# ntampellini/TSCoDe

Measured on AMD Instinct MI355X. Metric: conformers/sec, 100k x 50-atom prune_conformers pipeline (embed -> clash mask -> RMSD prune), higher is better.
Workload: dtype f64

## Files before the change

### tscode_amd/csrc/adjacent.hip

```cpp
#include "host.hpp"
#include "call.hpp"
#include "embed_transform.hpp"
#include "scan_kernels.hpp"
#include "gather_rows.hpp"
#include "prune_api.hpp"
#include "group_filter.hpp"
#include "csearch_kernels.hpp"
#include "tfd_kernels.hpp"
#include "moi_kernels.hpp"
#include "host_order.hpp"
#include "trimolecular.hpp"
#include "embed_prune_plan.hpp"

#include <memory>


extern "C" __attribute__((visibility("default"))) int tsc_greedy_group_filter_dev(tsc_ctx *c, const double *poses, const int32_t *group_off_dev, int n_groups,
                                                                             int64_t n_poses, int n_atoms, double rmsd_thr, uint8_t *accepted) {
    TSC_API_GUARD_BEGIN
    TSC_REQUIRE(c && poses && group_off_dev && accepted, "tsc_greedy_group_filter_dev: null argument");
    TSC_REQUIRE(n_groups >= 0 && n_poses >= 0 && n_atoms > 0 && rmsd_thr > 0, "bad sizes");
    if (n_groups == 0 || n_poses == 0) return 0;
    DeviceGuard guard(c->device);
    Scratch s(c);
    double *G;
    TSC_TRY(s.get(size_t(n_poses), &G));
    hipLaunchKernelGGL(k_greedy_group_filter, dim3(n_groups), dim3(256), 0, c->stream, poses, group_off_dev, n_groups, n_atoms, rmsd_thr,
                       accepted, G);
    TSC_HIP(hipGetLastError());
    return 0;
    TSC_API_GUARD_END
}

extern "C" __attribute__((visibility("default"))) int tsc_greedy_group_filter(tsc_ctx *c, const double *poses, const int32_t *group_off, int n_groups, int n_atoms,
                                                                         double rmsd_thr, uint8_t *accepted) {
    TSC_API_GUARD_BEGIN
    TSC_REQUIRE(c && poses && group_off && accepted, "tsc_greedy_group_filter: null argument");
    TSC_REQUIRE(n_groups >= 0 && n_atoms > 0 && rmsd_thr > 0, "bad sizes");
    if (n_groups == 0) return 0;
    TSC_REQUIRE(group_off[0] == 0, "group_off must start at 0");
    for (int g = 0; g < n_groups; ++g)
        TSC_REQUIRE(group_off[g + 1] >= group_off[g] && group_off[g + 1] - group_off[g] <= GF_MAX_GROUP,
                    "group %d: sizes must be in [0, %d]", g, GF_MAX_GROUP);
    const int64_t n_poses = group_off[n_groups];
    if (n_poses == 0) return 0;
    HostCall h(c);
    double *d_poses;
    int32_t *d_off;
    uint8_t *d_acc;
    TSC_TRY(h.in(poses, size_t(n_poses) * n_atoms * 3, &d_poses));
    TSC_TRY(h.in(group_off, size_t(n_groups) + 1, &d_off));
    TSC_TRY(h.out(accepted, size_t(n_poses), &d_acc));
    TSC_TRY(tsc_greedy_group_filter_dev(c, d_poses, d_off, n_groups, n_poses, n_atoms, rmsd_thr, d_acc));
    return h.finish();
    TSC_API_GUARD_END
}


static int csearch_args(int n_atoms, int n_tors, int64_t n_cand, double thresh, int64_t max_clashes, CsearchArgs *a) {
    TSC_REQUIRE(n_atoms > 0 && n_tors >= 0 && n_cand >= 0, "bad sizes (%d atoms, %d torsions, %lld candidates)", n_atoms, n_tors, (long long)n_cand);
    TSC_REQUIRE(n_atoms <= 65535 && torsion_lists_bytes(n_tors, n_atoms) + csearch_wave_bytes(n_atoms) <= 150 * 1024,
                "%d atoms x %d torsions exceed the LDS staging of the csearch kernels", n_atoms, n_tors);
    a->n = n_atoms, a->n_tors = n_tors, a->n_cand = n_cand;
    a->sq_bound = clash_sq_bound(thresh), a->max_clashes = max_clashes;
    return 0;
}

static int csearch_waves(int n_atoms, int n_tors, size_t *lds) {
    int w = 4;
    while (w > 1 && torsion_lists_bytes(n_tors, n_atoms) + w * csearch_wave_bytes(n_atoms) > 150 * 1024) w >>= 1;
    *lds = torsion_lists_bytes(n_tors, n_atoms) + w * csearch_wave_bytes(n_atoms);
    return w;
}

static int check_torsions(const int32_t *torsions, int n_tors, int n_atoms) {
    for (int t = 0; t < n_tors; ++t)
        for (int q = 0; q < 4; ++q)
            TSC_REQUIRE(torsions[4 * t + q] >= 0 && torsions[4 * t + q] < n_atoms, "torsion %d: atom index %d out of range", t, torsions[4 * t + q]);
    return 0;
}

extern "C" __attribute__((visibility("default"))) int tsc_csearch_rotate_dev(tsc_ctx *c, const double *coords, int n_atoms, const int32_t *torsions,
                                                                             const uint8_t *masks, int n_tors, const int32_t *angles, int64_t n_cand,
                                                                             double thresh, int64_t max_clashes, double *out, int32_t *rotated_bonds) {
    TSC_API_GUARD_BEGIN
    TSC_REQUIRE(c && coords && out && rotated_bonds && torsions && masks && angles, "tsc_csearch_rotate_dev: null argument");
    CsearchArgs a;
    TSC_TRY(csearch_args(n_atoms, n_tors, n_cand, thresh, max_clashes, &a));
    if (n_cand == 0) return 0;
    DeviceGuard guard(c->device);
    size_t lds;
    const int waves = csearch_waves(n_atoms, n_tors, &lds);
    TSC_TRY(lds_attribute(&k_csearch_rotate, lds));
    hipLaunchKernelGGL(k_csearch_rotate, dim3(grid_for(n_cand, waves, 256 * 8)), dim3(64 * waves), lds, c->stream, a, coords, torsions, masks, angles, out,
                       rotated_bonds);
    TSC_HIP(hipGetLastError());
    return 0;
    TSC_API_GUARD_END
}

extern "C" __attribute__((visibility("default"))) int tsc_csearch_rotate(tsc_ctx *c, const double *coords, int n_atoms, const int32_t *torsions,
                                                                         const uint8_t *masks, int n_tors, const int32_t *angles, int64_t n_cand,
                                                                         double thresh, int64_t max_clashes, double *out, int32_t *rotated_bonds) {
    TSC_API_GUARD_BEGIN
    TSC_REQUIRE(c && coords && out && rotated_bonds && (n_tors == 0 || (torsions && masks && angles)), "tsc_csearch_rotate: null argument");
    TSC_REQUIRE(n_atoms > 0 && n_tors >= 0 && n_cand >= 0, "bad sizes");
    TSC_TRY(check_torsions(torsions, n_tors, n_atoms));
    if (n_cand == 0) return 0;
    HostCall h(c);
    double *d_coords, *d_out;
    int32_t *d_tors, *d_angles, *d_rb;
    uint8_t *d_masks;
    TSC_TRY(h.in(coords, size_t(n_atoms) * 3, &d_coords));
    TSC_TRY(h.in(torsions, size_t(n_tors) * 4, &d_tors));
    TSC_TRY(h.in(masks, size_t(n_tors) * n_atoms, &d_masks));
    TSC_TRY(h.in(angles, size_t(n_cand) * n_tors, &d_angles));
    TSC_TRY(h.out(out, size_t(n_cand) * n_atoms * 3, &d_out));
    TSC_TRY(h.out(rotated_bonds, size_t(n_cand), &d_rb));
    TSC_TRY(tsc_csearch_rotate_dev(c, d_coords, n_atoms, d_tors, d_masks, n_tors, d_angles, n_cand, thresh, max_clashes, d_out, d_rb));
    return h.finish();
    TSC_API_GUARD_END
}

static int csearch_multi_sets(int n_atoms, const int32_t *set_off, int n_sets, int *t_widest) {
    TSC_REQUIRE(n_atoms > 0 && n_sets > 0 && set_off && set_off[0] == 0, "bad sizes (%d atoms, %d torsion sets; set_off must start at 0)", n_atoms, n_sets);
    int widest = 0;
    for (int k = 0; k < n_sets; ++k) {
        const int t = set_off[k + 1] - set_off[k];
        TSC_REQUIRE(t >= 0, "torsion set %d: set_off must not decrease", k);
        TSC_REQUIRE(n_atoms <= 65535 && torsion_lists_bytes(t, n_atoms) + csearch_wave_bytes(n_atoms) <= 150 * 1024,
                    "torsion set %d: %d atoms x %d torsions exceed the LDS staging of the csearch kernels", k, n_atoms, t);
        widest = std::max(widest, t);
    }
    *t_widest = widest;
    return 0;
}

extern "C" __attribute__((visibility("default"))) int tsc_csearch_multi_plan(const int32_t *cand_start, int64_t n_cand, const int32_t *start_set, int n_starts,
                                                                             const int32_t *set_off, int n_sets, int n_atoms, int32_t *items,
                                                                             int64_t items_cap, int64_t *n_items) {
    TSC_API_GUARD_BEGIN
    TSC_REQUIRE(n_items && (n_cand == 0 || cand_start) && (n_starts == 0 || start_set), "tsc_csearch_multi_plan: null argument");
    TSC_REQUIRE(n_cand >= 0 && n_cand < INT32_MAX && n_starts >= 0, "bad sizes (%lld candidates, %d starts)", (long long)n_cand, n_starts);
    int widest;
    TSC_TRY(csearch_multi_sets(n_atoms, set_off, n_sets, &widest));
    for (int s = 0; s < n_starts; ++s) TSC_REQUIRE(start_set[s] >= 0 && start_set[s] < n_sets, "start %d: torsion set %d out of range", s, start_set[s]);
    size_t lds;
    const int waves = csearch_waves(n_atoms, widest, &lds);
    int64_t count = 0;
    for (int64_t lo = 0; lo < n_cand;) {
        const int s = cand_start[lo];
        TSC_REQUIRE(s >= 0 && s < n_starts && (lo == 0 || s >= cand_start[lo - 1]), "candidate %lld: start %d out of range or out of order", (long long)lo, s);
        const int k = start_set[s];
        int64_t hi = lo + 1;
        while (hi < n_cand && hi - lo < waves && cand_start[hi] >= 0 && cand_start[hi] < n_starts && cand_start[hi] >= cand_start[hi - 1] &&
               start_set[cand_start[hi]] == k)
            ++hi;
        if (items) {
            TSC_REQUIRE(count < items_cap, "tsc_csearch_multi_plan: more than %lld work items", (long long)items_cap);
            items[4 * count] = int32_t(lo), items[4 * count + 1] = int32_t(hi), items[4 * count + 2] = set_off[k], items[4 * count + 3] = set_off[k + 1] - set_off[k];
        }
        ++count, lo = hi;
    }
    *n_items = count;
    return 0;
    TSC_API_GUARD_END
}

extern "C" __attribute__((visibility("default"))) int tsc_csearch_rotate_multi_dev(tsc_ctx *c, const double *starts, int n_atoms, const int32_t *torsions,
                                                                                   const uint8_t *masks, const int32_t *set_off, int n_sets,
                                                                                   const int32_t *angles, int t_max, const int32_t *cand_start,
                                                                                   const int32_t *cand_row, int64_t n_cand, const int32_t *items,
                                                                                   int64_t n_items, double thresh, int64_t max_clashes, double *out,
                                                                                   int32_t *rotated_bonds) {
    TSC_API_GUARD_BEGIN
    TSC_REQUIRE(c && set_off, "tsc_csearch_rotate_multi_dev: null argument");
    int widest;
    TSC_TRY(csearch_multi_sets(n_atoms, set_off, n_sets, &widest));
    TSC_REQUIRE(t_max >= widest && n_items >= 0 && n_items <= n_cand, "bad sizes (table %d wide, widest set %d; %lld work items, %lld candidates)", t_max,
                widest, (long long)n_items, (long long)n_cand);
    CsearchMultiArgs ma;
    TSC_TRY(csearch_args(n_atoms, widest, n_items, thresh, max_clashes, &ma.a));
    TSC_REQUIRE(n_cand < INT32_MAX, "too many candidates");
    if (n_cand == 0) return 0;
    TSC_REQUIRE(starts && out && rotated_bonds && cand_start && cand_row && items && (widest == 0 || (torsions && masks && angles)),
                "tsc_csearch_rotate_multi_dev: null argument");
    DeviceGuard guard(c->device);
    size_t lds;
    const int waves = csearch_waves(n_atoms, widest, &lds);
    ma.t_max = t_max, ma.lists_bytes = torsion_lists_bytes(widest, n_atoms);
    TSC_TRY(lds_attribute(&k_csearch_rotate_multi, lds));
    hipLaunchKernelGGL(k_csearch_rotate_multi, dim3(grid_for(n_items, 1, 256 * 8)), dim3(64 * waves), lds, c->stream, ma, starts, torsions, masks, angles,
                       cand_start, cand_row, items, out, rotated_bonds);
    TSC_HIP(hipGetLastError());
    return 0;
    TSC_API_GUARD_END
}

extern "C" __attribute__((visibility("default"))) int tsc_csearch_rotate_multi(tsc_ctx *c, const double *starts, int n_starts, int n_atoms, const int32_t *torsions,
                                                                               const uint8_t *masks, const int32_t *set_off, int n_sets,
                                                                               const int32_t *start_set, const int32_t *angles, int64_t n_rows, int t_max,
                                                                               const int32_t *cand_start, const int32_t *cand_row, int64_t n_cand,
                                                                               double thresh, int64_t max_clashes, double *out, int32_t *rotated_bonds) {
    TSC_API_GUARD_BEGIN
    TSC_REQUIRE(c && set_off && (n_cand == 0 || (starts && start_set && cand_start && cand_row && out && rotated_bonds)),
                "tsc_csearch_rotate_multi: null argument");
    TSC_REQUIRE(n_starts >= 0 && n_rows >= 0 && n_rows < INT32_MAX && n_cand >= 0 && t_max >= 0, "bad sizes");
    int64_t n_items = 0;
    TSC_TRY(tsc_csearch_multi_plan(cand_start, n_cand, start_set, n_starts, set_off, n_sets, n_atoms, nullptr, 0, &n_items));
    const int n_tors = set_off[n_sets];
    TSC_REQUIRE(n_tors == 0 || (torsions && masks), "tsc_csearch_rotate_multi: null argument");
    TSC_TRY(check_torsions(torsions, n_tors, n_atoms));
    for (int64_t m = 0; m < n_cand; ++m) TSC_REQUIRE(cand_row[m] >= 0 && cand_row[m] < n_rows, "candidate %lld: angle row %d out of range", (long long)m, cand_row[m]);
    if (n_cand == 0) return 0;
    TSC_REQUIRE(n_rows * t_max == 0 || angles, "tsc_csearch_rotate_multi: null argument");
    std::vector<int32_t> items(size_t(n_items) * 4);
    TSC_TRY(tsc_csearch_multi_plan(cand_start, n_cand, start_set, n_starts, set_off, n_sets, n_atoms, items.data(), n_items, &n_items));
    HostCall h(c);
    double *d_starts, *d_out;
    int32_t *d_tors, *d_angles, *d_cs, *d_cr, *d_items, *d_rb;
    uint8_t *d_masks;
    TSC_TRY(h.in(starts, size_t(n_starts) * n_atoms * 3, &d_starts));
    TSC_TRY(h.in(torsions, size_t(n_tors) * 4, &d_tors));
    TSC_TRY(h.in(masks, size_t(n_tors) * n_atoms, &d_masks));
    TSC_TRY(h.in(angles, size_t(n_rows) * t_max, &d_angles));
    TSC_TRY(h.in(cand_start, size_t(n_cand), &d_cs));
    TSC_TRY(h.in(cand_row, size_t(n_cand), &d_cr));
    TSC_TRY(h.in(items.data(), items.size(), &d_items));
    TSC_TRY(h.out(out, size_t(n_cand) * n_atoms * 3, &d_out));
    TSC_TRY(h.out(rotated_bonds, size_t(n_cand), &d_rb));
    TSC_TRY(tsc_csearch_rotate_multi_dev(c, d_starts, n_atoms, d_tors, d_masks, set_off, n_sets, d_angles, t_max, d_cs, d_cr, n_cand, d_items, n_items, thresh,
                                         max_clashes, d_out, d_rb));
    return h.finish();
    TSC_API_GUARD_END
}

extern "C" __attribute__((visibility("default"))) int tsc_csearch_select_dev(tsc_ctx *c, const double *cand, const int32_t *rotated_bonds, int n_atoms,
                                                                             const int32_t *seg_off, const int32_t *seg_start, const int32_t *seg_a0, int n_seg,
                                                                             int n_out, int64_t max_tries, int32_t *kept_count, int32_t *done,
                                                                             int32_t *rows_consumed, double *kept_rows, int64_t capacity,
                                                                             int64_t *n_kept_host) {
    TSC_API_GUARD_BEGIN
    TSC_REQUIRE(c && n_kept_host, "tsc_csearch_select_dev: null argument");
    TSC_REQUIRE(n_atoms > 0 && n_seg >= 0 && capacity >= 0, "bad sizes (%d atoms, %d segments, room for %lld rows)", n_atoms, n_seg, (long long)capacity);
    *n_kept_host = 0;
    if (n_seg == 0) return 0;
    TSC_REQUIRE(cand && rotated_bonds && seg_off && seg_start && seg_a0 && kept_count && done && rows_consumed && (capacity == 0 || kept_rows),
                "tsc_csearch_select_dev: null argument");
    DeviceGuard guard(c->device);
    Scratch s(c);
    int32_t *seg_kept, *total;
    TSC_TRY(s.get(size_t(n_seg), &seg_kept));
    TSC_TRY(s.get(1, &total));
    hipLaunchKernelGGL(k_csearch_select, dim3(grid_for(n_seg, 4, INT32_MAX)), dim3(256), 0, c->stream, rotated_bonds, seg_off, seg_start, seg_a0, n_seg, n_out,
                       (long long)max_tries, kept_count, done, rows_consumed, seg_kept);
    hipLaunchKernelGGL(k_csearch_compact, dim3(grid_for(n_seg, 4, INT32_MAX)), dim3(256), 0, c->stream, cand, rotated_bonds, seg_off, (const int32_t *)seg_kept,
                       n_seg, n_atoms * 3, (long long)capacity, kept_rows, total);
    TSC_HIP(hipGetLastError());
    int32_t kept = 0;
    TSC_TRY(read_i32(c, total, &kept));
    TSC_REQUIRE(kept <= capacity, "tsc_csearch_select_dev: %d rows kept, room for %lld (the rows past it were not written)", kept, (long long)capacity);
    *n_kept_host = kept;
    return 0;
    TSC_API_GUARD_END
}

extern "C" __attribute__((visibility("default"))) int tsc_rotate_dihedral(tsc_ctx *c, const double *coords, int64_t n_structs, int n_atoms, const int32_t *torsion,
                                                                          const uint8_t *mask, const double *angles, double *out) {
    TSC_API_GUARD_BEGIN
    TSC_REQUIRE(c && coords && torsion && mask && angles && out, "tsc_rotate_dihedral: null argument");
    TSC_REQUIRE(n_structs >= 0 && n_atoms > 0, "bad sizes");
    TSC_REQUIRE(out != coords, "tsc_rotate_dihedral: out must not alias coords");
    for (int q = 1; q <= 2; ++q) TSC_REQUIRE(torsion[q] >= 0 && torsion[q] < n_atoms, "torsion index %d out of range", torsion[q]);
    if (n_structs == 0) return 0;
    HostCall h(c);
    double *d_c, *d_o, *d_a;
    uint8_t *d_m;
    TSC_TRY(h.in(coords, size_t(n_structs) * n_atoms * 3, &d_c));
    TSC_TRY(h.in(angles, size_t(n_structs), &d_a));
    TSC_TRY(h.in(mask, size_t(n_atoms), &d_m));
    TSC_TRY(h.out(out, size_t(n_structs) * n_atoms * 3, &d_o));
    hipLaunchKernelGGL(k_rotate_dihedral, dim3(grid_for(n_structs * n_atoms, 256)), dim3(256), 0, c->stream, (const double *)d_c, n_structs, n_atoms, int(torsion[1]),
                       int(torsion[2]), (const uint8_t *)d_m, (const double *)d_a, d_o);
    TSC_HIP(hipGetLastError());
    return h.finish();
    TSC_API_GUARD_END
}

extern "C" __attribute__((visibility("default"))) int tsc_torsion_comp_check(tsc_ctx *c, const double *coords, int64_t n_structs, int n_atoms,
                                                                             const int32_t *torsion, const uint8_t *mask, double thresh,
                                                                             int64_t max_clashes, int32_t *ok) {
    TSC_API_GUARD_BEGIN
    TSC_REQUIRE(c && coords && torsion && mask && ok, "tsc_torsion_comp_check: null argument");
    CsearchArgs a;
    TSC_TRY(csearch_args(n_atoms, 1, n_structs, thresh, max_clashes, &a));
    TSC_TRY(check_torsions(torsion, 1, n_atoms));
    if (n_structs == 0) return 0;
    HostCall h(c);
    double *d_coords;
    int32_t *d_tors, *d_ok;
    uint8_t *d_mask;
    TSC_TRY(h.in(coords, size_t(n_structs) * n_atoms * 3, &d_coords));
    TSC_TRY(h.in(torsion, size_t(4), &d_tors));
    TSC_TRY(h.in(mask, size_t(n_atoms), &d_mask));
    TSC_TRY(h.out(ok, size_t(n_structs), &d_ok));
    size_t lds;
    const int waves = csearch_waves(n_atoms, 1, &lds);
    TSC_TRY(lds_attribute(&k_torsion_comp_check, lds));
    hipLaunchKernelGGL(k_torsion_comp_check, dim3(grid_for(n_structs, waves, 256 * 8)), dim3(64 * waves), lds, c->stream, a, (const double *)d_coords,
                       (const int32_t *)d_tors, (const uint8_t *)d_mask, d_ok);
    TSC_HIP(hipGetLastError());
    return h.finish();
    TSC_API_GUARD_END
}


extern "C" __attribute__((visibility("default"))) int tsc_torsion_fingerprints(tsc_ctx *c, const double *coords, int64_t n_structs, int n_atoms,
                                                                               const int32_t *quads, int n_quads, float *out) {
    TSC_API_GUARD_BEGIN
    TSC_REQUIRE(c && coords && quads && out, "tsc_torsion_fingerprints: null argument");
    TSC_REQUIRE(n_structs >= 0 && n_atoms > 0 && n_quads >= 0, "bad sizes");
    for (int q = 0; q < 4 * n_quads; ++q) TSC_REQUIRE(quads[q] >= 0 && quads[q] < n_atoms, "quadruplet atom index %d out of range", quads[q]);
    if (n_structs == 0 || n_quads == 0) return 0;
    HostCall h(c);
    double *d_coords;
    int32_t *d_quads;
    float *d_out;
    TSC_TRY(h.in(coords, size_t(n_structs) * n_atoms * 3, &d_coords));
    TSC_TRY(h.in(quads, size_t(n_quads) * 4, &d_quads));
    TSC_TRY(h.out(out, size_t(n_structs) * n_quads, &d_out));
    hipLaunchKernelGGL(k_torsion_fingerprints, dim3(grid_for(n_structs * n_quads, 256, 256 * 8)), dim3(256), 0, c->stream, (const double *)d_coords,
                       n_structs, n_atoms, (const int32_t *)d_quads, n_quads, d_out);
    TSC_HIP(hipGetLastError());
    return h.finish();
    TSC_API_GUARD_END
}

extern "C" __attribute__((visibility("default"))) int tsc_tfd_first_similar(tsc_ctx *c, const float *tf, int64_t n_structs, int n_quads, int64_t d,
                                                                            int64_t k, int64_t num_active, double thresh, int32_t *first) {
    TSC_API_GUARD_BEGIN
    TSC_REQUIRE(c && tf && first, "tsc_tfd_first_similar: null argument");
    if (n_structs == 0) return 0;
    TSC_REQUIRE(n_structs >= 0 && n_quads >= 0 && d > 0 && k > 0 && num_active >= 0 && num_active <= n_structs && d * k <= n_structs,
                "bad pass geometry (n = %lld, d = %lld, k = %lld, active = %lld)", (long long)n_structs, (long long)d, (long long)k, (long long)num_active);
    TSC_REQUIRE(n_structs < INT32_MAX, "too many structures");
    if (n_structs == 0) return 0;
    HostCall h(c);
    float *d_tf;
    int32_t *d_first;
    TSC_TRY(h.in(tf, size_t(n_structs) * n_quads, &d_tf));
    TSC_TRY(h.out(first, size_t(n_structs), &d_first));
    hipLaunchKernelGGL(k_tfd_first_similar, dim3(grid_for(n_structs, 4, 256 * 16)), dim3(256), 0, c->stream, (const float *)d_tf, n_structs, n_quads, d, k,
                       num_active, thresh, d_first);
    TSC_HIP(hipGetLastError());
    return h.finish();
    TSC_API_GUARD_END
}

extern "C" __attribute__((visibility("default"))) int tsc_host_graph_step(const int64_t *rel_i, const int64_t *rel_j, const int64_t *chunk_ptr,
                                                                          const int64_t *chunk_off, const int64_t *chunk_len, int64_t n_chunks,
                                                                          int64_t n_total, uint8_t *keep) {
    TSC_API_GUARD_BEGIN
    TSC_REQUIRE(rel_i && rel_j && chunk_ptr && chunk_off && chunk_len && keep && n_chunks >= 0 && n_total >= 0, "tsc_host_graph_step: bad argument");
    int64_t longest = 0;
    for (int64_t c = 0; c < n_chunks; ++c) {
        TSC_REQUIRE(chunk_ptr[c + 1] >= chunk_ptr[c] && chunk_off[c] >= 0 && chunk_len[c] >= 0 && chunk_off[c] + chunk_len[c] <= n_total,
                    "chunk %lld: bad bounds", (long long)c);
        for (int64_t q = chunk_ptr[c]; q < chunk_ptr[c + 1]; ++q)
            TSC_REQUIRE(rel_i[q] >= 0 && rel_i[q] < chunk_len[c] && rel_j[q] >= 0 && rel_j[q] < chunk_len[c] && rel_i[q] != rel_j[q],
                        "match %lld lies outside its chunk", (long long)q);
        longest = std::max(longest, chunk_len[c]);
    }
    std::vector<int32_t> index_of(size_t(longest), -1);
    for (int64_t c = 0; c < n_chunks; ++c)
        tsc_host::graph_step_chunk(rel_i + chunk_ptr[c], rel_j + chunk_ptr[c], chunk_ptr[c + 1] - chunk_ptr[c], chunk_off[c], keep, index_of);
    return 0;
    TSC_API_GUARD_END
}


extern "C" __attribute__((visibility("default"))) int tsc_inertia_moments(tsc_ctx *c, const double *structures, int64_t n_structs, int n_atoms,
                                                                          const double *masses, double *out) {
    TSC_API_GUARD_BEGIN
    TSC_REQUIRE(c && structures && masses && out && n_structs >= 0 && n_atoms > 0, "tsc_inertia_moments: bad argument");
    if (n_structs == 0) return 0;
    HostCall h(c);
    double *d_s, *d_m, *d_o;
    TSC_TRY(h.in(structures, size_t(n_structs) * n_atoms * 3, &d_s));
    TSC_TRY(h.in(masses, size_t(n_atoms), &d_m));
    TSC_TRY(h.out(out, size_t(n_structs) * 3, &d_o));
    hipLaunchKernelGGL(k_inertia_moments, dim3(grid_for(n_structs, 256, 256 * 8)), dim3(256), 0, c->stream, (const double *)d_s, n_structs, n_atoms,
                       (const double *)d_m, d_o);
    TSC_HIP(hipGetLastError());
    return h.finish();
    TSC_API_GUARD_END
}

extern "C" __attribute__((visibility("default"))) int tsc_moi_first_similar(tsc_ctx *c, const double *moments, int64_t n_structs, double max_deviation,
                                                                            int32_t *first) {
    TSC_API_GUARD_BEGIN
    TSC_REQUIRE(c && moments && first && n_structs >= 0 && n_structs < INT32_MAX, "tsc_moi_first_similar: bad argument");
    if (n_structs == 0) return 0;
    HostCall h(c);
    double *d_m;
    int32_t *d_f;
    TSC_TRY(h.in(moments, size_t(n_structs) * 3, &d_m));
    TSC_TRY(h.out(first, size_t(n_structs), &d_f));
    hipLaunchKernelGGL(k_moi_first_similar, dim3(grid_for(n_structs, 4, 256 * 16)), dim3(256), 0, c->stream, (const double *)d_m, n_structs, max_deviation, d_f);
    TSC_HIP(hipGetLastError());
    return h.finish();
    TSC_API_GUARD_END
}

extern "C" __attribute__((visibility("default"))) int tsc_embed_scores(tsc_ctx *c, const double *structures, int64_t n_structs, int n_atoms,
                                                                       const int32_t *indices, const double *distances, int n_c, float *scores,
                                                                       double *fitness_error) {
    TSC_API_GUARD_BEGIN
    TSC_REQUIRE(c && structures && indices && distances && scores && fitness_error && n_structs >= 0 && n_atoms > 0 && n_c >= 0, "tsc_embed_scores: bad argument");
    for (int64_t q = 0; q < n_structs * n_c * 2; ++q) TSC_REQUIRE(indices[q] >= 0 && indices[q] < n_atoms, "constrained index %d out of range", indices[q]);
    if (n_structs == 0) return 0;
    HostCall h(c);
    double *d_s, *d_d, *d_e;
    int32_t *d_i;
    float *d_sc;
    TSC_TRY(h.in(structures, size_t(n_structs) * n_atoms * 3, &d_s));
    TSC_TRY(h.in(indices, size_t(n_structs) * n_c * 2, &d_i));
    TSC_TRY(h.in(distances, size_t(n_structs) * n_c, &d_d));
    TSC_TRY(h.out(scores, size_t(n_structs), &d_sc));
    TSC_TRY(h.out(fitness_error, size_t(n_structs), &d_e));
    hipLaunchKernelGGL(k_embed_scores, dim3(grid_for(n_structs, 256, 256 * 8)), dim3(256), 0, c->stream, (const double *)d_s, n_structs, n_atoms,
                       (const int32_t *)d_i, (const double *)d_d, n_c, d_sc, d_e);
    TSC_HIP(hipGetLastError());
    return h.finish();
    TSC_API_GUARD_END
}


extern "C" __attribute__((visibility("default"))) int tsc_string_embed_params_dev(tsc_ctx *c, const double *p1, const double *p2, const double *ref_vec,
                                                                                  const double *mol_vec, const int32_t *conf_pair, int64_t n_sites,
                                                                                  const double *angles, int n_angles, double *rot, double *pos,
                                                                                  int32_t *conf_idx) {
    TSC_API_GUARD_BEGIN
    TSC_REQUIRE(c && p1 && p2 && ref_vec && mol_vec && conf_pair && angles && rot && pos && conf_idx, "tsc_string_embed_params_dev: null argument");
    TSC_REQUIRE(n_sites >= 0 && n_angles >= 0, "bad sizes");
    if (n_sites == 0 || n_angles == 0) return 0;
    DeviceGuard guard(c->device);
    hipLaunchKernelGGL(k_string_embed_params, dim3(grid_for(n_sites * n_angles, 256, 256 * 8)), dim3(256), 0, c->stream, p1, p2, ref_vec, mol_vec,
                       conf_pair, n_sites, angles, n_angles, rot, pos, conf_idx);
    TSC_HIP(hipGetLastError());
    return 0;
    TSC_API_GUARD_END
}

extern "C" __attribute__((visibility("default"))) int tsc_string_embed_params(tsc_ctx *c, const double *p1, const double *p2, const double *ref_vec,
                                                                              const double *mol_vec, const int32_t *conf_pair, int64_t n_sites,
                                                                              const double *angles, int n_angles, double *rot, double *pos,
                                                                              int32_t *conf_idx) {
    TSC_API_GUARD_BEGIN
    TSC_REQUIRE(c && p1 && p2 && ref_vec && mol_vec && conf_pair && angles && rot && pos && conf_idx, "tsc_string_embed_params: null argument");
    TSC_REQUIRE(n_sites >= 0 && n_angles >= 0, "bad sizes");
    if (n_sites == 0 || n_angles == 0) return 0;
    HostCall h(c);
    double *d_p1, *d_p2, *d_rv, *d_mv, *d_ang, *d_rot, *d_pos;
    int32_t *d_cp, *d_ci;
    const size_t N = size_t(n_sites) * n_angles;
    TSC_TRY(h.in(p1, size_t(n_sites) * 3, &d_p1));
    TSC_TRY(h.in(p2, size_t(n_sites) * 3, &d_p2));
    TSC_TRY(h.in(ref_vec, size_t(n_sites) * 3, &d_rv));
    TSC_TRY(h.in(mol_vec, size_t(n_sites) * 3, &d_mv));
    TSC_TRY(h.in(conf_pair, size_t(n_sites) * 2, &d_cp));
    TSC_TRY(h.in(angles, size_t(n_angles), &d_ang));
    TSC_TRY(h.out(rot, N * 18, &d_rot));
    TSC_TRY(h.out(pos, N * 6, &d_pos));
    TSC_TRY(h.out(conf_idx, N * 2, &d_ci));
    TSC_TRY(tsc_string_embed_params_dev(c, d_p1, d_p2, d_rv, d_mv, d_cp, n_sites, d_ang, n_angles, d_rot, d_pos, d_ci));
    return h.finish();
    TSC_API_GUARD_END
}

extern "C" __attribute__((visibility("default"))) int tsc_cyclical_embed_params(tsc_ctx *c, const double *start, const double *end,
                                                                                const double *direction, const double *pivot, const double *meanpoint,
                                                                                const double *r0, const double *r1, const int32_t *n_reactive,
                                                                                const double *angle, int64_t n, double *rot, double *pos) {
    TSC_API_GUARD_BEGIN
    TSC_REQUIRE(c && start && end && direction && pivot && meanpoint && r0 && r1 && n_reactive && angle && rot && pos, "tsc_cyclical_embed_params: null argument");
    TSC_REQUIRE(n >= 0, "bad size");
    for (int64_t q = 0; q < n; ++q) TSC_REQUIRE(n_reactive[q] == 1 || n_reactive[q] == 2, "row %lld: n_reactive must be 1 or 2", (long long)q);
    if (n == 0) return 0;
    HostCall h(c);
    const double *host[7] = {start, end, direction, pivot, meanpoint, r0, r1};
    double *dev[7], *d_angle, *d_rot, *d_pos;
    int32_t *d_nr;
    for (int i = 0; i < 7; ++i) TSC_TRY(h.in(host[i], size_t(n) * 3, &dev[i]));
    TSC_TRY(h.in(n_reactive, size_t(n), &d_nr));
    TSC_TRY(h.in(angle, size_t(n), &d_angle));
    TSC_TRY(h.out(rot, size_t(n) * 9, &d_rot));
    TSC_TRY(h.out(pos, size_t(n) * 3, &d_pos));
    hipLaunchKernelGGL(k_cyclical_embed_params, dim3(grid_for(n, 256, 256 * 8)), dim3(256), 0, c->stream, (const double *)dev[0], (const double *)dev[1],
                       (const double *)dev[2], (const double *)dev[3], (const double *)dev[4], (const double *)dev[5], (const double *)dev[6],
                       (const int32_t *)d_nr, (const double *)d_angle, n, d_rot, d_pos);
    TSC_HIP(hipGetLastError());
    return h.finish();
    TSC_API_GUARD_END
}


static int launch_tfd_greedy(tsc_ctx *c, Scratch &s, const float *d_tf, int64_t n, int T, double thresh, uint8_t *d_acc, int32_t *d_list, int32_t *d_nk) {
    TSC_REQUIRE(T <= 12288, "fingerprints of %d torsions: the greedy filter takes up to 12288", T);
    uint8_t *d_flags;
    unsigned long long *d_sim;
    float *d_kfp;
    TSC_TRY(s.get(size_t(TG_SUPER) + TG_WORDS * sizeof(unsigned long long), &d_flags));
    TSC_TRY(s.get(size_t(TG_SUPER) * TG_WORDS, &d_sim));
    TSC_TRY(s.get(std::max<size_t>(size_t(n) * T, 1), &d_kfp));
    int32_t *d_nk_before;
    TSC_TRY(s.get(1, &d_nk_before));
    unsigned long long *d_nz = reinterpret_cast<unsigned long long *>(d_flags + TG_SUPER);
    const size_t lds_pairs = 64 * T <= 12288 ? size_t(64) * std::max(T, 1) * sizeof(float) : 0;
    TSC_HIP(hipMemsetAsync(d_nk, 0, sizeof(int32_t), c->stream));
    for (int64_t base = 0; base < n; base += TG_SUPER) {
        const int nc = int(std::min<int64_t>(TG_SUPER, n - base));
        TSC_HIP(hipMemsetAsync(d_flags, 0, size_t(TG_SUPER) + TG_WORDS * sizeof(unsigned long long), c->stream));
        if (base > 0)
            hipLaunchKernelGGL(k_tfd_greedy_prior, dim3(ceil_div(nc, 256), 64), dim3(256), 0, c->stream, d_tf, base, nc, T, thresh, (const float *)d_kfp,
                               (const int32_t *)d_nk, d_flags);
        hipLaunchKernelGGL(k_tfd_greedy_pairs, dim3(TG_WORDS, ceil_div(nc, 256)), dim3(256), lds_pairs, c->stream, d_tf, base, nc, T, thresh, d_sim, d_nz);
        hipLaunchKernelGGL(k_tfd_greedy_replay, dim3(1), dim3(64), 0, c->stream, (const unsigned long long *)d_sim, (const unsigned long long *)d_nz, base, nc,
                           (const uint8_t *)d_flags, d_acc, d_list, d_nk, d_nk_before);
        if (base + TG_SUPER < n && T > 0)
            hipLaunchKernelGGL(k_tfd_greedy_keep, dim3(1), dim3(256), 0, c->stream, d_tf, T, (const int32_t *)d_list, (const int32_t *)d_nk_before,
                               (const int32_t *)d_nk, d_kfp);
    }
    TSC_HIP(hipGetLastError());
    return 0;
}

extern "C" __attribute__((visibility("default"))) int tsc_tfd_greedy_filter(tsc_ctx *c, const float *tf, int64_t n_structs, int n_quads, double thresh,
                                                                            uint8_t *accepted, int64_t *n_kept) {
    TSC_API_GUARD_BEGIN
    TSC_REQUIRE(c && tf && accepted, "tsc_tfd_greedy_filter: null argument");
    TSC_REQUIRE(n_structs >= 0 && n_structs < INT32_MAX && n_quads >= 0, "bad sizes");
    if (n_kept) *n_kept = 0;
    if (n_structs == 0) return 0;
    int32_t nk = 0;
    HostCall h(c);
    float *d_tf;
    uint8_t *d_acc;
    int32_t *d_list, *d_nk;
    TSC_TRY(h.in(tf, std::max<size_t>(size_t(n_structs) * n_quads, 1), &d_tf));
    TSC_TRY(h.out(accepted, size_t(n_structs), &d_acc));
    TSC_TRY(h.scratch().get(size_t(n_structs), &d_list));
    TSC_TRY(h.scratch().get(1, &d_nk));
    TSC_TRY(launch_tfd_greedy(c, h.scratch(), d_tf, n_structs, n_quads, thresh, d_acc, d_list, d_nk));
    TSC_TRY(h.fetch(&nk, d_nk, 1));
    TSC_TRY(h.finish());
    if (n_kept) *n_kept = nk;
    return 0;
    TSC_API_GUARD_END
}

struct EmbedFiltered {
    int32_t n_pass = 0, n_kept = 0;
    double *structs = nullptr;
    int32_t *act = nullptr;
    int32_t *act2 = nullptr;
    const int32_t *ci = nullptr;
    const double *rot = nullptr, *pos = nullptr;
};

template <typename Filter>
static int embed_filter_front(tsc_ctx *c, HostCall &h, const double *d_frags, const FragTable &ft, const int64_t *frag_off, const int32_t *n_atoms,
                              const int32_t *n_conf, const int32_t *d_ci, const double *d_rot, const double *d_pos, int64_t N, double clash_thresh,
                              int64_t max_clashes, uint8_t *clash_ok, uint8_t *kept, EmbedFiltered *f, Filter filter) {
    hipStream_t st = c->stream;
    Scratch &s = h.scratch();
    const int n = ft.n_total;
    uint8_t *d_mask, *d_kept_full, *d_acc;
    int32_t *bsum, *act, *pos_scan, *total, *act2, *total2;
    TSC_TRY(s.get(size_t(N), &d_mask));
    TSC_TRY(h.out(kept, size_t(N), &d_kept_full));
    TSC_TRY(s.get(scan_bsum_count(N), &bsum));
    TSC_TRY(s.get(size_t(N), &act));
    TSC_TRY(s.get(size_t(N) + 1, &pos_scan));
    TSC_TRY(s.get(1, &total));
    TSC_TRY(s.get(size_t(N), &act2));
    TSC_TRY(s.get(1, &total2));
    TSC_TRY(tsc_embed_clash_mask_dev(c, d_frags, frag_off, n_atoms, n_conf, ft.n_mols, d_ci, d_rot, d_pos, N, clash_thresh, max_clashes, d_mask, nullptr));
    TSC_TRY(scan_mask(st, d_mask, N, bsum, pos_scan, act, nullptr, total));
    TSC_TRY(h.fetch(clash_ok, d_mask, size_t(N)));
    TSC_HIP(hipMemsetAsync(d_kept_full, 0, size_t(N), st));
    f->act = act, f->act2 = act2;
    TSC_TRY(read_i32(c, total, &f->n_pass));
    const int32_t n_pass = f->n_pass;
    if (n_pass > 0) {
        double *d_structs;
        TSC_TRY(s.get(size_t(n_pass) * n * 3, &d_structs));
        TSC_TRY(s.get(size_t(n_pass), &d_acc));
        hipLaunchKernelGGL(k_transform, dim3(grid_for(n_pass, TR_POSES, 256 * 64)), dim3(256), transform_lds_bytes(ft.n_mols), st, d_frags, ft, d_ci, d_rot, d_pos,
                           (const int32_t *)act, int64_t(n_pass), d_structs, (const int32_t *)nullptr, 0, (double *)nullptr, (const int32_t *)nullptr);
        TSC_HIP(hipGetLastError());
        f->structs = d_structs;
        TSC_TRY(filter(d_structs, n_pass, pos_scan, total, d_acc));
        hipLaunchKernelGGL(k_scatter_flags, dim3(grid_for(n_pass, 256, 1024)), dim3(256), 0, st, (const uint8_t *)d_acc, (const int32_t *)act, (const int32_t *)total,
                           d_kept_full);
        TSC_TRY(scan_mask(st, d_acc, n_pass, bsum, nullptr, act2, nullptr, total2));
        TSC_TRY(read_i32(c, total2, &f->n_kept));
    }
    return 0;
}

static int embed_filter_fetch(tsc_ctx *c, HostCall &h, int n, const EmbedFiltered &f, double *poses, int64_t poses_capacity, int64_t *n_kept_out) {
    if (poses && f.n_kept > 0) {
        double *d_out;
        TSC_REQUIRE(f.n_kept <= poses_capacity, "poses holds %lld rows, %d poses were kept", (long long)poses_capacity, f.n_kept);
        TSC_TRY(h.scratch().get(size_t(f.n_kept) * n * 3, &d_out));
        TSC_TRY(launch_gather_rows(c->stream, f.structs, f.act2, f.n_kept, n * 3, nullptr, n * 3, d_out));
        TSC_TRY(h.fetch(poses, d_out, size_t(f.n_kept) * n * 3));
    }
    TSC_TRY(h.finish());
    *n_kept_out = f.n_kept;
    return 0;
}

template <typename Filter>
static int embed_filter_run(tsc_ctx *c, HostCall &h, const double *d_frags, const FragTable &ft, const int64_t *frag_off, const int32_t *n_atoms,
                            const int32_t *n_conf, const int32_t *d_ci, const double *d_rot, const double *d_pos, int64_t N, double clash_thresh,
                            int64_t max_clashes, uint8_t *clash_ok, uint8_t *kept, double *poses, int64_t poses_capacity, int64_t *n_pass_out,
                            int64_t *n_kept_out, Filter filter) {
    EmbedFiltered f;
    const int rc = embed_filter_front(c, h, d_frags, ft, frag_off, n_atoms, n_conf, d_ci, d_rot, d_pos, N, clash_thresh, max_clashes, clash_ok, kept, &f, filter);
    *n_pass_out = f.n_pass;
    TSC_TRY(rc);
    return embed_filter_fetch(c, h, ft.n_total, f, poses, poses_capacity, n_kept_out);
}

extern "C" __attribute__((visibility("default"))) int tsc_string_embed(tsc_ctx *c, const double *frags, const int64_t *frag_off, const int32_t *n_atoms,
                                                                       const int32_t *n_conf, const double *p1, const double *p2, const double *ref_vec,
                                                                       const double *mol_vec, const int32_t *conf_pair, int64_t n_sites, const double *angles,
                                                                       int n_angles, double clash_thresh, int64_t max_clashes, const int32_t *quads, int n_quads,
                                                                       double tfd_thresh, uint8_t *clash_ok, uint8_t *kept, double *poses,
                                                                       int64_t poses_capacity, int64_t *n_pass, int64_t *n_kept) {
    TSC_API_GUARD_BEGIN
    TSC_REQUIRE(c && frags && frag_off && n_atoms && n_conf && p1 && p2 && ref_vec && mol_vec && conf_pair && angles && clash_ok && kept && n_pass && n_kept,
                "tsc_string_embed: null argument");
    TSC_REQUIRE(n_sites >= 0 && n_angles >= 0 && n_quads >= 0 && (n_quads == 0 || quads), "bad sizes");
    const int64_t N = n_sites * n_angles;
    TSC_REQUIRE(N < INT32_MAX, "too many candidates");
    *n_pass = *n_kept = 0;
    if (N == 0) return 0;
    FragTable ft;
    TSC_TRY(make_frag_table(frag_off, n_atoms, n_conf, 2, &ft));
    for (int64_t q = 0; q < n_sites; ++q)
        TSC_REQUIRE(conf_pair[2 * q] >= 0 && conf_pair[2 * q] < n_conf[0] && conf_pair[2 * q + 1] >= 0 && conf_pair[2 * q + 1] < n_conf[1],
                    "site %lld: conformer index out of range", (long long)q);
    for (int q = 0; q < 4 * n_quads; ++q) TSC_REQUIRE(quads[q] >= 0 && quads[q] < ft.n_total, "quadruplet atom index %d out of range", quads[q]);
    HostCall h(c);
    Scratch &s = h.scratch();
    double *d_frags, *d_p1, *d_p2, *d_rv, *d_mv, *d_ang, *d_rot, *d_pos;
    int32_t *d_cp, *d_ci, *d_quads = nullptr;
    TSC_TRY(h.in(frags, size_t(frags_total_doubles(frag_off, n_atoms, n_conf, 2)), &d_frags));
    TSC_TRY(h.in(p1, size_t(n_sites) * 3, &d_p1));
    TSC_TRY(h.in(p2, size_t(n_sites) * 3, &d_p2));
    TSC_TRY(h.in(ref_vec, size_t(n_sites) * 3, &d_rv));
    TSC_TRY(h.in(mol_vec, size_t(n_sites) * 3, &d_mv));
    TSC_TRY(h.in(conf_pair, size_t(n_sites) * 2, &d_cp));
    TSC_TRY(h.in(angles, size_t(n_angles), &d_ang));
    if (n_quads) TSC_TRY(h.in(quads, size_t(n_quads) * 4, &d_quads));
    TSC_TRY(s.get(size_t(N) * 18, &d_rot));
    TSC_TRY(s.get(size_t(N) * 6, &d_pos));
    TSC_TRY(s.get(size_t(N) * 2, &d_ci));
    TSC_TRY(tsc_string_embed_params_dev(c, d_p1, d_p2, d_rv, d_mv, d_cp, n_sites, d_ang, n_angles, d_rot, d_pos, d_ci));
    const int n = ft.n_total;
    auto filter = [&](const double *d_structs, int32_t np, const int32_t *, const int32_t *, uint8_t *d_acc) -> int {
        float *d_tf;
        int32_t *d_list, *d_nk;
        TSC_TRY(s.get(std::max<size_t>(size_t(np) * n_quads, 1), &d_tf));
        TSC_TRY(s.get(size_t(np), &d_list));
        TSC_TRY(s.get(1, &d_nk));
        if (n_quads)
            hipLaunchKernelGGL(k_torsion_fingerprints, dim3(grid_for(int64_t(np) * n_quads, 256, 256 * 8)), dim3(256), 0, c->stream, d_structs, int64_t(np), n,
                               (const int32_t *)d_quads, n_quads, d_tf);
        TSC_HIP(hipGetLastError());
        return launch_tfd_greedy(c, s, d_tf, int64_t(np), n_quads, tfd_thresh, d_acc, d_list, d_nk);
    };
    return embed_filter_run(c, h, d_frags, ft, frag_off, n_atoms, n_conf, d_ci, d_rot, d_pos, N, clash_thresh, max_clashes, clash_ok, kept, poses, poses_capacity,
                            n_pass, n_kept, filter);
    TSC_API_GUARD_END
}

extern "C" __attribute__((visibility("default"))) int tsc_cyclical_embed(tsc_ctx *c, const double *frags, const int64_t *frag_off, const int32_t *n_atoms,
                                                                         const int32_t *n_conf, int n_mols, const double *start, const double *end,
                                                                         const double *direction, const double *pivot, const double *meanpoint, const double *r0,
                                                                         const double *r1, const int32_t *n_reactive, const double *angle, const int32_t *conf_idx,
                                                                         int64_t n_poses, const int32_t *group_off, int n_groups, double clash_thresh,
                                                                         int64_t max_clashes, double rmsd_thr, uint8_t *clash_ok, uint8_t *kept, double *poses,
                                                                         int64_t poses_capacity, int64_t *n_pass, int64_t *n_kept) {
    TSC_API_GUARD_BEGIN
    TSC_REQUIRE(c && frags && frag_off && n_atoms && n_conf && start && end && direction && pivot && meanpoint && r0 && r1 && n_reactive && angle && conf_idx &&
                    group_off && clash_ok && kept && n_pass && n_kept,
                "tsc_cyclical_embed: null argument");
    TSC_REQUIRE(n_poses >= 0 && n_poses < INT32_MAX && n_groups >= 0 && rmsd_thr > 0, "bad sizes");
    *n_pass = *n_kept = 0;
    if (n_poses == 0) return 0;
    FragTable ft;
    TSC_TRY(make_frag_table(frag_off, n_atoms, n_conf, n_mols, &ft));
    const int64_t rows = n_poses * n_mols;
    for (int64_t q = 0; q < rows; ++q) {
        TSC_REQUIRE(n_reactive[q] == 1 || n_reactive[q] == 2, "row %lld: n_reactive must be 1 or 2", (long long)q);
        TSC_REQUIRE(conf_idx[q] >= 0 && conf_idx[q] < n_conf[q % n_mols], "row %lld: conformer index out of range", (long long)q);
    }
    TSC_REQUIRE(n_groups > 0 && group_off[0] == 0 && group_off[n_groups] == n_poses, "group_off must run from 0 to n_poses");
    for (int g = 0; g < n_groups; ++g)
        TSC_REQUIRE(group_off[g + 1] >= group_off[g] && group_off[g + 1] - group_off[g] <= GF_MAX_GROUP, "group %d: sizes must be in [0, %d]", g, GF_MAX_GROUP);
    HostCall h(c);
    Scratch &s = h.scratch();
    const double *host[7] = {start, end, direction, pivot, meanpoint, r0, r1};
    double *d_frags, *dev[7], *d_angle, *d_rot, *d_pos;
    int32_t *d_nr, *d_ci, *d_goff, *d_goff_pass;
    TSC_TRY(h.in(frags, size_t(frags_total_doubles(frag_off, n_atoms, n_conf, n_mols)), &d_frags));
    for (int i = 0; i < 7; ++i) TSC_TRY(h.in(host[i], size_t(rows) * 3, &dev[i]));
    TSC_TRY(h.in(n_reactive, size_t(rows), &d_nr));
    TSC_TRY(h.in(angle, size_t(rows), &d_angle));
    TSC_TRY(h.in(conf_idx, size_t(rows), &d_ci));
    TSC_TRY(h.in(group_off, size_t(n_groups) + 1, &d_goff));
    TSC_TRY(s.get(size_t(n_groups) + 1, &d_goff_pass));
    TSC_TRY(s.get(size_t(rows) * 9, &d_rot));
    TSC_TRY(s.get(size_t(rows) * 3, &d_pos));
    hipLaunchKernelGGL(k_cyclical_embed_params, dim3(grid_for(rows, 256, 256 * 8)), dim3(256), 0, c->stream, (const double *)dev[0], (const double *)dev[1],
                       (const double *)dev[2], (const double *)dev[3], (const double *)dev[4], (const double *)dev[5], (const double *)dev[6],
                       (const int32_t *)d_nr, (const double *)d_angle, rows, d_rot, d_pos);
    TSC_HIP(hipGetLastError());
    const int n = ft.n_total;
    auto filter = [&](const double *d_structs, int32_t np, const int32_t *pos_scan, const int32_t *total, uint8_t *d_acc) -> int {
        hipLaunchKernelGGL(k_group_offsets_after_filter, dim3(grid_for(n_groups + 1, 256, 1024)), dim3(256), 0, c->stream, (const int32_t *)d_goff, n_groups, pos_scan,
                           n_poses, total, d_goff_pass);
        TSC_HIP(hipGetLastError());
        return tsc_greedy_group_filter_dev(c, d_structs, d_goff_pass, n_groups, np, n, rmsd_thr, d_acc);
    };
    return embed_filter_run(c, h, d_frags, ft, frag_off, n_atoms, n_conf, d_ci, d_rot, d_pos, n_poses, clash_thresh, max_clashes, clash_ok, kept, poses,
                            poses_capacity, n_pass, n_kept, filter);
    TSC_API_GUARD_END
}

static int check_group_slab_sizes(int64_t n_groups, int n_angles, double rmsd_thr) {
    TSC_REQUIRE(n_angles >= 1 && n_angles <= GF_MAX_GROUP, "%d angle sets per group: must be in [1, %d]", n_angles, GF_MAX_GROUP);
    TSC_REQUIRE(n_groups >= 0 && n_groups < INT32_MAX / n_angles, "%lld groups of %d poses: too many candidates", (long long)n_groups, n_angles);
    TSC_REQUIRE(rmsd_thr > 0, "bad sizes");
    return 0;
}
static int check_group_slab_records(const int32_t *n_conf, int n_mols, const int32_t *n_reactive, const int32_t *conf_idx, int64_t n_groups) {
    for (int64_t q = 0; q < n_groups * n_mols; ++q) {
        TSC_REQUIRE(n_reactive[q] == 1 || n_reactive[q] == 2, "group %lld, molecule %d: n_reactive must be 1 or 2", (long long)(q / n_mols), int(q % n_mols));
        TSC_REQUIRE(conf_idx[q] >= 0 && conf_idx[q] < n_conf[q % n_mols], "group %lld, molecule %d: conformer index out of range", (long long)(q / n_mols),
                    int(q % n_mols));
    }
    return 0;
}

static int cyclical_groups_front(tsc_ctx *c, HostCall &h, std::vector<int32_t> &goff, const double *d_frags, const FragTable &ft, const int64_t *frag_off,
                                 const int32_t *n_atoms, const int32_t *n_conf, const double *const host[7], const int32_t *n_reactive, const int32_t *conf_idx,
                                 const double *angles, int64_t n_groups, int n_angles, double clash_thresh, int64_t max_clashes, double rmsd_thr,
                                 uint8_t *clash_ok, uint8_t *kept, EmbedFiltered *f) {
    const int n_mols = ft.n_mols;
    const int64_t items = n_groups * n_mols, n_poses = n_groups * n_angles, rows = n_poses * n_mols;
    goff.resize(size_t(n_groups) + 1);
    for (int64_t g = 0; g <= n_groups; ++g) goff[size_t(g)] = int32_t(g * n_angles);
    Scratch &s = h.scratch();
    double *dev[7], *d_angles, *d_rot, *d_pos;
    int32_t *d_nr, *d_cg, *d_ci, *d_goff, *d_goff_pass;
    for (int i = 0; i < 7; ++i) TSC_TRY(h.in(host[i], size_t(items) * 3, &dev[i]));
    TSC_TRY(h.in(n_reactive, size_t(items), &d_nr));
    TSC_TRY(h.in(conf_idx, size_t(items), &d_cg));
    TSC_TRY(h.in(angles, size_t(n_angles) * n_mols, &d_angles));
    TSC_TRY(h.in(goff.data(), size_t(n_groups) + 1, &d_goff));
    TSC_TRY(s.get(size_t(n_groups) + 1, &d_goff_pass));
    TSC_TRY(s.get(size_t(rows) * 9, &d_rot));
    TSC_TRY(s.get(size_t(rows) * 3, &d_pos));
    TSC_TRY(s.get(size_t(rows), &d_ci));
    hipLaunchKernelGGL(k_cyclical_embed_group_params, dim3(grid_for(ceil_div(n_groups, int64_t(64 / n_mols)), CGP_WAVES, 768)), dim3(64 * CGP_WAVES), 0, c->stream,
                       (const double *)dev[0], (const double *)dev[1], (const double *)dev[2], (const double *)dev[3], (const double *)dev[4],
                       (const double *)dev[5], (const double *)dev[6], (const int32_t *)d_nr, (const int32_t *)d_cg, (const double *)d_angles, n_groups, n_mols,
                       n_angles, d_rot, d_pos, d_ci);
    TSC_HIP(hipGetLastError());
    f->ci = d_ci, f->rot = d_rot, f->pos = d_pos;
    const int n = ft.n_total;
    const int ng = int(n_groups);
    auto filter = [&](const double *d_structs, int32_t np, const int32_t *pos_scan, const int32_t *total, uint8_t *d_acc) -> int {
        hipLaunchKernelGGL(k_group_offsets_after_filter, dim3(grid_for(ng + 1, 256, 1024)), dim3(256), 0, c->stream, (const int32_t *)d_goff, ng, pos_scan, n_poses,
                           total, d_goff_pass);
        TSC_HIP(hipGetLastError());
        return tsc_greedy_group_filter_dev(c, d_structs, d_goff_pass, ng, np, n, rmsd_thr, d_acc);
    };
    return embed_filter_front(c, h, d_frags, ft, frag_off, n_atoms, n_conf, d_ci, d_rot, d_pos, n_poses, clash_thresh, max_clashes, clash_ok, kept, f, filter);
}

extern "C" __attribute__((visibility("default"))) int tsc_cyclical_embed_groups(tsc_ctx *c, const double *frags, const int64_t *frag_off, const int32_t *n_atoms,
                                                                                const int32_t *n_conf, int n_mols, const double *start, const double *end,
                                                                                const double *direction, const double *pivot, const double *meanpoint,
                                                                                const double *r0, const double *r1, const int32_t *n_reactive,
                                                                                const int32_t *conf_idx, const double *angles, int64_t n_groups, int n_angles,
                                                                                double clash_thresh, int64_t max_clashes, double rmsd_thr, uint8_t *clash_ok,
                                                                                uint8_t *kept, double *poses, int64_t poses_capacity, int64_t *n_pass,
                                                                                int64_t *n_kept) {
    TSC_API_GUARD_BEGIN
    TSC_REQUIRE(c && frags && frag_off && n_atoms && n_conf && start && end && direction && pivot && meanpoint && r0 && r1 && n_reactive && conf_idx && angles &&
                    clash_ok && kept && n_pass && n_kept,
                "tsc_cyclical_embed_groups: null argument");
    TSC_REQUIRE(n_mols == 2 || n_mols == 3, "tsc_cyclical_embed_groups: %d molecules, the cyclical embed takes 2 or 3", n_mols);
    TSC_TRY(check_group_slab_sizes(n_groups, n_angles, rmsd_thr));
    *n_pass = *n_kept = 0;
    if (n_groups == 0) return 0;
    FragTable ft;
    TSC_TRY(make_frag_table(frag_off, n_atoms, n_conf, n_mols, &ft));
    TSC_TRY(check_group_slab_records(n_conf, n_mols, n_reactive, conf_idx, n_groups));
    std::vector<int32_t> goff;
    HostCall h(c);
    const double *host[7] = {start, end, direction, pivot, meanpoint, r0, r1};
    double *d_frags;
    TSC_TRY(h.in(frags, size_t(frags_total_doubles(frag_off, n_atoms, n_conf, n_mols)), &d_frags));
    EmbedFiltered f;
    const int rc = cyclical_groups_front(c, h, goff, d_frags, ft, frag_off, n_atoms, n_conf, host, n_reactive, conf_idx, angles, n_groups, n_angles, clash_thresh,
                                         max_clashes, rmsd_thr, clash_ok, kept, &f);
    *n_pass = f.n_pass;
    TSC_TRY(rc);
    return embed_filter_fetch(c, h, ft.n_total, f, poses, poses_capacity, n_kept);
    TSC_API_GUARD_END
}


static thread_local float g_trimolecular_ms = -1.f;

extern "C" __attribute__((visibility("default"))) int tsc_trimolecular_groups_timings(tsc_ctx *c, float *ms) {
    TSC_API_GUARD_BEGIN
    TSC_REQUIRE(c && ms, "tsc_trimolecular_groups_timings: null argument");
    *ms = g_trimolecular_ms;
    return 0;
    TSC_API_GUARD_END
}

extern "C" __attribute__((visibility("default"))) int tsc_trimolecular_groups(
    tsc_ctx *c, const double *frags, const int64_t *frag_off, const int32_t *n_atoms, const int32_t *n_conf, const int32_t *reactive, const int32_t *n_reactive,
    const int64_t *reactive_cumnums, const int32_t *n_rows, const int32_t *conf, const double *pivot, const double *meanpoint, const int64_t *cumnums,
    const double *tri_poly, const double *tri_cost, const double *directions, const uint8_t *mask, const int64_t *base, int64_t n_triples, int64_t n_groups,
    double *blocks, int64_t *group_ids, int32_t *best) {
    TSC_API_GUARD_BEGIN
    TSC_REQUIRE(c && frags && frag_off && n_atoms && n_conf && reactive && n_reactive && reactive_cumnums && n_rows, "tsc_trimolecular_groups: null argument");
    TSC_REQUIRE(n_triples >= 0 && n_groups >= 0 && n_groups < INT32_MAX, "tsc_trimolecular_groups: %lld triples, %lld groups", (long long)n_triples,
                (long long)n_groups);
    FragTable ft;
    TSC_TRY(make_frag_table(frag_off, n_atoms, n_conf, 3, &ft));
    TriTables tb;
    memset(&tb, 0, sizeof(tb));
    const int64_t *row = reactive_cumnums;
    for (int m = 0; m < 3; ++m) {
        tb.frag_off[m] = frag_off[m], tb.n_atoms[m] = n_atoms[m], tb.n_reactive[m] = n_reactive[m], tb.n_rows[m] = n_rows[m];
        TSC_REQUIRE(n_reactive[m] == 1 || n_reactive[m] == 2, "tsc_trimolecular_groups: molecule %d has %d reactive atoms, must be 1 or 2", m, n_reactive[m]);
        for (int k = 0; k < n_reactive[m]; ++k) {
            TSC_REQUIRE(reactive[2 * m + k] >= 0 && reactive[2 * m + k] < n_atoms[m], "tsc_trimolecular_groups: reactive atom %d of molecule %d with %d atoms",
                        reactive[2 * m + k], m, n_atoms[m]);
            tb.reactive[m][k] = reactive[2 * m + k];
        }
        TSC_REQUIRE(n_rows[m] >= 0 && n_rows[m] <= TG_MAX_ROWS, "tsc_trimolecular_groups: molecule %d has %d reactive_cumnums rows, at most %d are taken", m,
                    n_rows[m], TG_MAX_ROWS);
        for (int r = 0; r < n_rows[m]; ++r, row += 2) {
            TSC_REQUIRE(row[0] >= 0 && row[0] < n_atoms[m], "tsc_trimolecular_groups: reactive_cumnums row %d of molecule %d names atom %lld of %d", r, m,
                        (long long)row[0], n_atoms[m]);
            tb.row_atom[m][r] = int(row[0]), tb.row_cum[m][r] = row[1];
        }
    }
    g_trimolecular_ms = -1.f;
    if (n_triples == 0) {
        TSC_REQUIRE(n_groups == 0, "tsc_trimolecular_groups: %lld groups from no triple", (long long)n_groups);
        return 0;
    }
    TSC_REQUIRE(conf && pivot && meanpoint && cumnums && tri_poly && tri_cost && directions && mask && base, "tsc_trimolecular_groups: null argument");
    TSC_REQUIRE(n_groups == 0 || (blocks && group_ids && best), "tsc_trimolecular_groups: null output");
    int64_t running = 0;
    for (int64_t t = 0; t < n_triples; ++t) {
        TSC_REQUIRE(base[t] == running, "tsc_trimolecular_groups: triple %lld: base %lld, the orientation masks in front of it count %lld", (long long)t,
                    (long long)base[t], (long long)running);
        running += __builtin_popcount(mask[t]);
        for (int m = 0; m < 3; ++m)
            TSC_REQUIRE(conf[3 * t + m] >= 0 && conf[3 * t + m] < n_conf[m], "tsc_trimolecular_groups: triple %lld, molecule %d: conformer %d of %d",
                        (long long)t, m, conf[3 * t + m], n_conf[m]);
        if (!mask[t]) continue;
        for (int q = 0; q < 6; ++q) {
            bool found = false;
            for (int m = 0; m < 3 && !found; ++m)
                for (int r = 0; r < tb.n_rows[m] && !found; ++r) found = tb.row_cum[m][r] == cumnums[6 * t + q];
            TSC_REQUIRE(found, "tsc_trimolecular_groups: triple %lld: cumnum %lld of molecule %d's pivot is in no molecule's reactive_cumnums", (long long)t,
                        (long long)cumnums[6 * t + q], q / 2);
        }
    }
    TSC_REQUIRE(running == n_groups, "tsc_trimolecular_groups: the orientation masks count %lld groups, n_groups is %lld", (long long)running, (long long)n_groups);
    if (n_groups == 0) return 0;
    HostCall h(c);
    const size_t T = size_t(n_triples), G = size_t(n_groups);
    const double *d_frags, *d_pivot, *d_mean, *d_poly, *d_cost, *d_dir;
    const int32_t *d_conf;
    const int64_t *d_cum, *d_base;
    const uint8_t *d_mask;
    double *d_blocks;
    int64_t *d_ids;
    int32_t *d_best;
    TSC_TRY(h.in(frags, size_t(frags_total_doubles(frag_off, n_atoms, n_conf, 3)), &d_frags));
    TSC_TRY(h.in(conf, T * 3, &d_conf));
    TSC_TRY(h.in(pivot, T * 9, &d_pivot));
    TSC_TRY(h.in(meanpoint, T * 9, &d_mean));
    TSC_TRY(h.in(cumnums, T * 6, &d_cum));
    TSC_TRY(h.in(tri_poly, T * 9, &d_poly));
    TSC_TRY(h.in(tri_cost, T * 9, &d_cost));
    TSC_TRY(h.in(directions, T * 9, &d_dir));
    TSC_TRY(h.in(mask, T, &d_mask));
    TSC_TRY(h.in(base, T, &d_base));
    TSC_TRY(h.out(blocks, G * 3 * TG_RECORD, &d_blocks));
    TSC_TRY(h.out(group_ids, G * 6, &d_ids));
    TSC_TRY(h.out(best, G, &d_best));
    StageTimer tm(c);
    tm.begin();
    hipLaunchKernelGGL(k_trimolecular_groups, dim3(grid_for(n_triples, TG_WAVES, 512)), dim3(64 * TG_WAVES), 0, c->stream, d_frags, tb, d_conf, d_pivot, d_mean,
                       d_cum, d_poly, d_cost, d_dir, d_mask, d_base, n_triples, d_blocks, d_ids, d_best);
    const hipError_t launched = hipGetLastError();
    if (launched == hipSuccess) tm.end(&g_trimolecular_ms);
    TSC_HIP(launched);
    return h.finish();
    TSC_API_GUARD_END
}


struct tsc_embed_prune : Owned {
    using Owned::Owned;
    FragTable ft{};
    int64_t frag_off[MAX_MOLS] = {};
    int32_t n_atoms[MAX_MOLS] = {}, n_conf[MAX_MOLS] = {};
    int n_heavy = 0;
    double *frags = nullptr;
    int32_t *sel = nullptr;
    double *heavy = nullptr, *rot = nullptr, *pos = nullptr;
    int32_t *ci = nullptr;
    uint8_t *survived = nullptr;
    int64_t cap = 0, n_kept = 0, n_survived = 0;
    bool pruned = false;
};

static __global__ __launch_bounds__(256) void k_kept_candidates(const int32_t *__restrict__ act, const int32_t *__restrict__ act2, int n_kept,
                                                                int32_t *__restrict__ cand) {
    for (int r = blockIdx.x * 256 + threadIdx.x; r < n_kept; r += gridDim.x * 256) cand[r] = act[act2[r]];
}

static __global__ __launch_bounds__(256) void k_gather_rows_i32(const int32_t *__restrict__ src, const int32_t *__restrict__ idx, int64_t n_out, int row,
                                                                int32_t *__restrict__ dst) {
    const int64_t total = n_out * row;
    for (int64_t e = int64_t(blockIdx.x) * 256 + threadIdx.x; e < total; e += int64_t(gridDim.x) * 256) {
        const int64_t r = e / row;
        dst[e] = src[int64_t(idx[r]) * row + (e - r * row)];
    }
}

static int embed_prune_reserve(tsc_embed_prune *r, int64_t need) {
    tsc_ctx *c = r->ctx;
    const int64_t cap = ep_grown_capacity(r->cap, need);
    TSC_REQUIRE(cap >= 0, "tsc_embed_prune_add_groups: %lld kept poses are more than a prune takes (%lld)", (long long)need, (long long)EP_MAX_ROWS);
    if (cap == r->cap) return 0;
    const int nm = r->ft.n_mols;
    const size_t row_bytes[4] = {size_t(r->n_heavy) * 24, size_t(nm) * 72, size_t(nm) * 24, size_t(nm) * 4};
    void *old[4] = {r->heavy, r->rot, r->pos, r->ci}, *grown[4] = {nullptr, nullptr, nullptr, nullptr};
    int rc = 0;
    for (int i = 0; i < 4 && !rc; ++i) rc = r->take(size_t(cap) * row_bytes[i], &grown[i]);
    for (int i = 0; i < 4 && !rc; ++i)
        if (r->n_kept > 0 && hipMemcpyAsync(grown[i], old[i], size_t(r->n_kept) * row_bytes[i], hipMemcpyDeviceToDevice, c->stream) != hipSuccess)
            rc = fail(TSC_ERR_HIP, "tsc_embed_prune_add_groups: the copy into the grown buffers failed");
    void *const *gone = rc ? grown : old;
    for (int i = 0; i < 4; ++i) r->give_back(gone[i]);
    if (rc) return rc;
    r->heavy = static_cast<double *>(grown[0]), r->rot = static_cast<double *>(grown[1]), r->pos = static_cast<double *>(grown[2]);
    r->ci = static_cast<int32_t *>(grown[3]);
    r->cap = cap;
    return 0;
}

extern "C" __attribute__((visibility("default"))) int tsc_embed_prune_destroy(tsc_embed_prune *r) {
    TSC_API_GUARD_BEGIN
    return destroy_owned(r);
    TSC_API_GUARD_END
}

extern "C" __attribute__((visibility("default"))) int tsc_embed_prune_create(tsc_ctx *c, const double *frags, const int64_t *frag_off, const int32_t *n_atoms,
                                                                             const int32_t *n_conf, int n_mols, const int32_t *heavy_idx, int n_heavy,
                                                                             tsc_embed_prune **out) {
    TSC_API_GUARD_BEGIN
    TSC_REQUIRE(c && frags && frag_off && n_atoms && n_conf && heavy_idx && out, "tsc_embed_prune_create: null argument");
    *out = nullptr;
    TSC_REQUIRE(n_mols == 2 || n_mols == 3, "tsc_embed_prune_create: %d molecules, the cyclical embed takes 2 or 3", n_mols);
    FragTable ft;
    TSC_TRY(make_frag_table(frag_off, n_atoms, n_conf, n_mols, &ft));
    TSC_REQUIRE(n_heavy >= 1 && n_heavy <= ft.n_total, "tsc_embed_prune_create: %d heavy atoms of %d atoms: at least one, at most all", n_heavy, ft.n_total);
    std::vector<int32_t> sel(size_t(n_heavy) * 3);
    for (int a = 0; a < n_heavy; ++a) {
        TSC_REQUIRE(heavy_idx[a] >= 0 && heavy_idx[a] < ft.n_total, "tsc_embed_prune_create: heavy_idx[%d] = %d is not an atom of the %d", a, heavy_idx[a],
                    ft.n_total);
        TSC_REQUIRE(a == 0 || heavy_idx[a] > heavy_idx[a - 1], "tsc_embed_prune_create: heavy_idx[%d] = %d does not increase", a, heavy_idx[a]);
        for (int k = 0; k < 3; ++k) sel[size_t(a) * 3 + k] = heavy_idx[a] * 3 + k;
    }
    HostCall h(c);
    std::unique_ptr<tsc_embed_prune> run(new tsc_embed_prune(c));
    run->ft = ft, run->n_heavy = n_heavy;
    for (int m = 0; m < n_mols; ++m) run->frag_off[m] = frag_off[m], run->n_atoms[m] = n_atoms[m], run->n_conf[m] = n_conf[m];
    TSC_TRY(h.in(frags, size_t(frags_total_doubles(frag_off, n_atoms, n_conf, n_mols)), &run->frags));
    TSC_TRY(h.in(sel.data(), sel.size(), &run->sel));
    TSC_TRY(h.finish());
    run->take_blocks(h.scratch());
    c->owned.adopt(run.get());
    *out = run.release();
    return 0;
    TSC_API_GUARD_END
}

extern "C" __attribute__((visibility("default"))) int tsc_embed_prune_add_groups(tsc_embed_prune *r, const double *start, const double *end, const double *direction,
                                                                                 const double *pivot, const double *meanpoint, const double *r0, const double *r1,
                                                                                 const int32_t *n_reactive, const int32_t *conf_idx, const double *angles,
                                                                                 int64_t n_groups, int n_angles, double clash_thresh, int64_t max_clashes,
                                                                                 double rmsd_thr_filter, uint8_t *clash_ok, uint8_t *kept, int64_t *n_pass,
                                                                                 int64_t *n_kept) {
    TSC_API_GUARD_BEGIN
    TSC_REQUIRE(r && start && end && direction && pivot && meanpoint && r0 && r1 && n_reactive && conf_idx && angles && clash_ok && kept && n_pass && n_kept,
                "tsc_embed_prune_add_groups: null argument");
    if (r->pruned) return fail(TSC_ERR_STATE, "tsc_embed_prune_add_groups: the run has been pruned (tsc_embed_prune_run); a further slab needs a new run");
    TSC_TRY(check_group_slab_sizes(n_groups, n_angles, rmsd_thr_filter));
    *n_pass = *n_kept = 0;
    if (n_groups == 0) return 0;
    tsc_ctx *c = r->ctx;
    const int n_mols = r->ft.n_mols, n = r->ft.n_total;
    TSC_TRY(check_group_slab_records(r->n_conf, n_mols, n_reactive, conf_idx, n_groups));
    std::vector<int32_t> goff;
    HostCall h(c);
    const double *host[7] = {start, end, direction, pivot, meanpoint, r0, r1};
    EmbedFiltered f;
    const int rc = cyclical_groups_front(c, h, goff, r->frags, r->ft, r->frag_off, r->n_atoms, r->n_conf, host, n_reactive, conf_idx, angles, n_groups, n_angles,
                                         clash_thresh, max_clashes, rmsd_thr_filter, clash_ok, kept, &f);
    *n_pass = f.n_pass;
    TSC_TRY(rc);
    if (f.n_kept > 0) {
        TSC_TRY(embed_prune_reserve(r, r->n_kept + f.n_kept));
        int32_t *cand;
        TSC_TRY(h.scratch().get(size_t(f.n_kept), &cand));
        hipLaunchKernelGGL(k_kept_candidates, dim3(grid_for(f.n_kept, 256, 1024)), dim3(256), 0, c->stream, (const int32_t *)f.act, (const int32_t *)f.act2, f.n_kept,
                           cand);
        TSC_HIP(hipGetLastError());
        const int64_t at = r->n_kept;
        TSC_TRY(launch_gather_rows(c->stream, f.structs, f.act2, f.n_kept, n * 3, r->sel, r->n_heavy * 3, r->heavy + ep_row_offset(at, r->n_heavy * 3)));
        TSC_TRY(launch_gather_rows(c->stream, f.rot, cand, f.n_kept, n_mols * 9, nullptr, n_mols * 9, r->rot + ep_row_offset(at, n_mols * 9)));
        TSC_TRY(launch_gather_rows(c->stream, f.pos, cand, f.n_kept, n_mols * 3, nullptr, n_mols * 3, r->pos + ep_row_offset(at, n_mols * 3)));
        hipLaunchKernelGGL(k_gather_rows_i32, dim3(grid_for(int64_t(f.n_kept) * n_mols, 256, 1024)), dim3(256), 0, c->stream, f.ci, (const int32_t *)cand,
                           int64_t(f.n_kept), n_mols, r->ci + ep_row_offset(at, n_mols));
        TSC_HIP(hipGetLastError());
    }
    TSC_TRY(h.finish());
    r->n_kept += f.n_kept;
    *n_kept = f.n_kept;
    return 0;
    TSC_API_GUARD_END
}

extern "C" __attribute__((visibility("default"))) int tsc_embed_prune_count(tsc_embed_prune *r, int64_t *n_kept_total) {
    TSC_API_GUARD_BEGIN
    TSC_REQUIRE(r && n_kept_total, "tsc_embed_prune_count: null argument");
    *n_kept_total = r->n_kept;
    return 0;
    TSC_API_GUARD_END
}

extern "C" __attribute__((visibility("default"))) int tsc_embed_prune_run(tsc_embed_prune *r, double rmsd_thr, int mode, uint8_t *survived, tsc_pass_stats *stats,
                                                                          int *n_passes, int64_t *n_survived) {
    TSC_API_GUARD_BEGIN
    TSC_REQUIRE(r && n_survived && (survived || r->n_kept == 0), "tsc_embed_prune_run: null argument");
    TSC_REQUIRE(mode == 0 || mode == 1, "tsc_embed_prune_run: mode %d (0: reference-exact, 1: cache-free)", mode);
    TSC_REQUIRE(rmsd_thr > 0, "tsc_embed_prune_run: rmsd_thr = %g must be positive", rmsd_thr);
    *n_survived = 0;
    if (n_passes) *n_passes = 0;
    tsc_ctx *c = r->ctx;
    if (r->n_kept == 0) {
        r->pruned = true, r->n_survived = 0;
        return 0;
    }
    DeviceGuard guard(c->device);
    if (!r->survived) TSC_TRY(r->get(size_t(r->n_kept), &r->survived));
    r->pruned = true, r->n_survived = 0;
    TSC_TRY(tsc_prune_rmsd_dev(c, r->heavy, r->n_kept, r->n_heavy, rmsd_thr, mode, r->survived, stats, n_passes));
    TSC_HIP(hipMemcpyAsync(survived, r->survived, size_t(r->n_kept), hipMemcpyDeviceToHost, c->stream));
    TSC_HIP(hipStreamSynchronize(c->stream));
    int64_t count = 0;
    for (int64_t i = 0; i < r->n_kept; ++i) count += survived[i] != 0;
    r->n_survived = count;
    *n_survived = count;
    return 0;
    TSC_API_GUARD_END
}

extern "C" __attribute__((visibility("default"))) int tsc_embed_prune_poses(tsc_embed_prune *r, int which, double *poses, int64_t capacity) {
    TSC_API_GUARD_BEGIN
    TSC_REQUIRE(r && poses, "tsc_embed_prune_poses: null argument");
    TSC_REQUIRE(which == 0 || which == 1, "tsc_embed_prune_poses: which = %d (0: the survivors, 1: every kept pose)", which);
    if (which == 0 && !r->pruned) return fail(TSC_ERR_STATE, "tsc_embed_prune_poses: the survivors are known once tsc_embed_prune_run has run");
    const int64_t rows = which == 0 ? r->n_survived : r->n_kept;
    TSC_REQUIRE(capacity >= rows, "tsc_embed_prune_poses: poses holds %lld rows, %lld are asked for", (long long)capacity, (long long)rows);
    if (rows == 0) return 0;
    tsc_ctx *c = r->ctx;
    const int n = r->ft.n_total;
    HostCall h(c);
    Scratch &s = h.scratch();
    int32_t *act = nullptr;
    if (which == 0) {
        int32_t *bsum;
        TSC_TRY(s.get(scan_bsum_count(r->n_kept), &bsum));
        TSC_TRY(s.get(size_t(r->n_kept), &act));
        TSC_TRY(scan_mask(c->stream, r->survived, r->n_kept, bsum, nullptr, act, nullptr, nullptr));
    }
    double *d_out;
    TSC_TRY(s.get(size_t(rows) * n * 3, &d_out));
    hipLaunchKernelGGL(k_transform, dim3(grid_for(rows, TR_POSES, 256 * 64)), dim3(256), transform_lds_bytes(r->ft.n_mols), c->stream, (const double *)r->frags, r->ft,
                       (const int32_t *)r->ci, (const double *)r->rot, (const double *)r->pos, (const int32_t *)act, rows, d_out, (const int32_t *)nullptr, 0,
                       (double *)nullptr, (const int32_t *)nullptr);
    TSC_HIP(hipGetLastError());
    TSC_TRY(h.fetch(poses, (const double *)d_out, size_t(rows) * n * 3));
    return h.finish();
    TSC_API_GUARD_END
}
```

### tscode_amd/csrc/describe.hpp

```cpp
#pragma once
#include "descriptor.hpp"
#include "embed_clash.hpp"

namespace tsc {

__device__ inline void describe_from_lds(const double *s_q, const double *s_x, int pitch, int h, int nf0, int nf1, const double *__restrict__ bias,
                                         int ns, int S, int64_t i0, float *__restrict__ D, double *__restrict__ G, unsigned *__restrict__ dmax_bits) {
    const int T = 256 / S;
    const int sidx = threadIdx.x / T, sub = threadIdx.x - sidx * T;
    const bool mine = sidx < ns;
    double d[DW], g = 0.0;
#pragma unroll
    for (int k = 0; k < DW; ++k) d[k] = 0.0;
    if (mine) {
        const double *x = s_x + sidx * pitch;
        const double *q1 = s_q + KD * nf0;
        for (int a = sub; a < h; a += T) {
            const double n2 = x[3 * a] * x[3 * a] + x[3 * a + 1] * x[3 * a + 1] + x[3 * a + 2] * x[3 * a + 2];
            g += n2;
            if (a < nf0) {
                const double f = sqrt(n2);
#pragma unroll
                for (int k = 0; k < KD; ++k) d[k] = fma(s_q[k * nf0 + a], f, d[k]);
            }
            if (a < nf1) {
                const double f = feature(x, h, 1, a);
#pragma unroll
                for (int k = 0; k < KD; ++k) d[KD + k] = fma(q1[k * nf1 + a], f, d[KD + k]);
            }
        }
    }
    for (int off = T >> 1; off > 0; off >>= 1) {
#pragma unroll
        for (int k = 0; k < DW; ++k) d[k] += __shfl_xor(d[k], off);
        g += __shfl_xor(g, off);
    }
    float mx = 0.0f;
    if (mine && sub == 0) {
        float v[DW];
#pragma unroll
        for (int k = 0; k < DW; ++k) {
            v[(k % KD) * 2 + k / KD] = float(d[k] - bias[k]);
            mx = fmaxf(mx, fabsf(float(d[k] - bias[k])));
        }
        f32x4 *dst = reinterpret_cast<f32x4 *>(D + (i0 + sidx) * DW);
#pragma unroll
        for (int k = 0; k < DW / 4; ++k) dst[k] = f32x4{v[4 * k], v[4 * k + 1], v[4 * k + 2], v[4 * k + 3]};
        G[i0 + sidx] = g;
    }
    for (int off = 32; off > 0; off >>= 1) mx = fmaxf(mx, __shfl_xor(mx, off));
    if ((threadIdx.x & 63) == 0 && mx > __uint_as_float(__hip_atomic_load(dmax_bits, __ATOMIC_RELAXED, __HIP_MEMORY_SCOPE_AGENT)))
        atomicMax(dmax_bits, __float_as_uint(mx));
    if (__ballot(mine && sub == 0 && !(g < 1.7976931348623157e308)) != 0 && (threadIdx.x & 63) == 0) atomicMax(dmax_bits, NONFINITE_BITS);
}

inline __global__ __launch_bounds__(256) void k_descriptors(const double *__restrict__ heavy, int64_t n, int h, int nf0, int nf1,
                                                      const double *__restrict__ Q, const double *__restrict__ bias, float *__restrict__ D,
                                                      double *__restrict__ G, unsigned *__restrict__ dmax_bits, int S) {
    extern __shared__ __attribute__((aligned(16))) double s_mem[];
    const int h3 = h * 3, pitch = h3 | 1;
    double *s_q = s_mem, *s_x = s_mem + KD * (nf0 + nf1);
    for (int e = threadIdx.x; e < KD * (nf0 + nf1); e += 256) s_q[e] = Q[e];
    const int64_t i0 = int64_t(blockIdx.x) * S;
    const int ns = int(min<int64_t>(S, n - i0));
    const double *src = heavy + i0 * h3;
    for (int base = threadIdx.x; base < ns * h3; base += 256 * 8) {
        double v[8];
#pragma unroll
        for (int j = 0; j < 8; ++j) v[j] = (base + 256 * j < ns * h3) ? src[base + 256 * j] : 0.0;
#pragma unroll
        for (int j = 0; j < 8; ++j) {
            const int e = base + 256 * j;
            if (e < ns * h3) {
                const int row = e / h3;
                s_x[row * pitch + (e - row * h3)] = v[j];
            }
        }
    }
    __syncthreads();
    describe_from_lds(s_q, s_x, pitch, h, nf0, nf1, bias, ns, S, i0, D, G, dmax_bits);
}

inline __global__ __launch_bounds__(256) void k_transform_describe(const double *__restrict__ frags, FragTable ft, const int32_t *__restrict__ conf_idx,
                                                             const double *__restrict__ rot, const double *__restrict__ pos,
                                                             const int32_t *__restrict__ idx, double *__restrict__ out,
                                                             const int32_t *__restrict__ heavy_slot, int n_heavy, double *__restrict__ heavy_out,
                                                             const int32_t *__restrict__ n_out_dev, int nf0, int nf1, const double *__restrict__ Q,
                                                             const double *__restrict__ bias, float *__restrict__ D, double *__restrict__ G,
                                                             unsigned *__restrict__ dmax_bits, float *__restrict__ heavy32_out = nullptr) {
    extern __shared__ __attribute__((aligned(16))) double s_tr[];
    const int n = ft.n_total, nm = ft.n_mols, tid = threadIdx.x, pitch = (n_heavy * 3) | 1;
    const int pitch32 = heavy32_pitch(n_heavy), pad32 = pitch32 - 3 * n_heavy;
    const int64_t n_out = *n_out_dev;
    int64_t *sP = reinterpret_cast<int64_t *>(s_tr);
    double *sR = s_tr + TR_POSES, *sT = sR + TR_POSES * nm * 9;
    int *sC = reinterpret_cast<int *>(sT + TR_POSES * nm * 3);
    double *s_q = s_tr + (transform_lds_bytes(nm) + 15) / 16 * 2, *s_x = s_q + KD * (nf0 + nf1);
    for (int e = tid; e < KD * (nf0 + nf1); e += 256) s_q[e] = Q[e];
    for (int64_t r0 = int64_t(blockIdx.x) * TR_POSES; r0 < n_out; r0 += int64_t(gridDim.x) * TR_POSES) {
        const int np = int(min<int64_t>(TR_POSES, n_out - r0));
        if (tid < np) sP[tid] = int64_t(idx[r0 + tid]);
        __syncthreads();
        for (int q = tid; q < np * nm * 9; q += 256) {
            const int row = q / (nm * 9), w = q - row * nm * 9;
            sR[q] = rot[sP[row] * nm * 9 + w];
        }
        for (int q = tid; q < np * nm * 3; q += 256) {
            const int row = q / (nm * 3), w = q - row * nm * 3;
            sT[q] = pos[sP[row] * nm * 3 + w];
        }
        for (int q = tid; q < np * nm; q += 256) {
            const int row = q / nm, w = q - row * nm;
            sC[q] = conf_idx[sP[row] * nm + w];
        }
        __syncthreads();
        for (int e = tid; e < np * n; e += 256) {
            const int row = e / n, a = e - row * n;
            const int64_t r = r0 + row;
            double v[3];
            embed_atom_staged(frags, ft, sR, sT, sC, row, a, v);
            if (out) {
                double *o = out + (r * n + a) * 3;
                o[0] = v[0], o[1] = v[1], o[2] = v[2];
            }
            const int hs = heavy_slot[a];
            if (hs >= 0) {
                double *hv = heavy_out + (r * n_heavy + hs) * 3, *x = s_x + row * pitch + hs * 3;
                hv[0] = x[0] = v[0], hv[1] = x[1] = v[1], hv[2] = x[2] = v[2];
                if (heavy32_out) {
                    float *hf = heavy32_out + r * pitch32 + hs * 3;
                    hf[0] = float(v[0]), hf[1] = float(v[1]), hf[2] = float(v[2]);
                }
            }
        }
        if (heavy32_out)
            for (int e = tid; e < np * pad32; e += 256) heavy32_out[(r0 + e / pad32) * pitch32 + 3 * n_heavy + e % pad32] = 0.0f;
        __syncthreads();
        describe_from_lds(s_q, s_x, pitch, n_heavy, nf0, nf1, bias, np, TR_POSES, r0, D, G, dmax_bits);
        __syncthreads();
    }
}

inline size_t transform_describe_lds_bytes(int n_mols, int h) {
    return (transform_lds_bytes(n_mols) + 15) / 16 * 16 + (size_t(KD) * (n_features(h, 0) + n_features(h, 1)) + size_t(TR_POSES) * ((h * 3) | 1)) * sizeof(double);
}

}
```

### tscode_amd/csrc/embed.hip

```cpp
#include "host.hpp"
#include "call.hpp"
#include "embed_transform.hpp"
#include "embed_clash_kernels.hpp"
#include "scan_kernels.hpp"
#include "gather_rows.hpp"


extern "C" __attribute__((visibility("default"))) int tsc_transform_batch_dev(tsc_ctx *c, const double *frags, const int64_t *frag_off, const int32_t *n_atoms,
                                       const int32_t *n_conf, int n_mols, const int32_t *conf_idx, const double *rot,
                                       const double *pos, int64_t n_poses, double *out) {
    TSC_API_GUARD_BEGIN
    TSC_REQUIRE(c && frags && conf_idx && rot && pos && out, "tsc_transform_batch_dev: null argument");
    TSC_REQUIRE(n_poses >= 0, "negative n_poses");
    FragTable ft;
    TSC_TRY(make_frag_table(frag_off, n_atoms, n_conf, n_mols, &ft));
    if (n_poses == 0) return 0;
    DeviceGuard guard(c->device);
    hipLaunchKernelGGL(k_transform, dim3(grid_for(n_poses, TR_POSES, 256 * 64)), dim3(256), transform_lds_bytes(ft.n_mols), c->stream, frags, ft, conf_idx, rot,
                       pos, (const int32_t *)nullptr, n_poses, out, (const int32_t *)nullptr, 0, (double *)nullptr, (const int32_t *)nullptr);
    TSC_HIP(hipGetLastError());
    return 0;
    TSC_API_GUARD_END
}


extern "C" __attribute__((visibility("default"))) int tsc_transform_batch(tsc_ctx *c, const double *frags, const int64_t *frag_off, const int32_t *n_atoms,
                                   const int32_t *n_conf, int n_mols, const int32_t *conf_idx, const double *rot,
                                   const double *pos, int64_t n_poses, double *out) {
    TSC_API_GUARD_BEGIN
    TSC_REQUIRE(c && frags && conf_idx && rot && pos && out, "tsc_transform_batch: null argument");
    FragTable ft;
    TSC_TRY(make_frag_table(frag_off, n_atoms, n_conf, n_mols, &ft));
    TSC_REQUIRE(n_poses >= 0, "negative n_poses");
    for (int64_t i = 0; i < n_poses * n_mols; ++i)
        TSC_REQUIRE(conf_idx[i] >= 0 && conf_idx[i] < n_conf[i % n_mols], "conf_idx[%lld] out of range", (long long)i);
    if (n_poses == 0) return 0;
    HostCall h(c);
    double *d_frags, *d_rot, *d_pos, *d_out;
    int32_t *d_ci;
    TSC_TRY(h.in(frags, size_t(frags_total_doubles(frag_off, n_atoms, n_conf, n_mols)), &d_frags));
    TSC_TRY(h.in(conf_idx, size_t(n_poses) * n_mols, &d_ci));
    TSC_TRY(h.in(rot, size_t(n_poses) * n_mols * 9, &d_rot));
    TSC_TRY(h.in(pos, size_t(n_poses) * n_mols * 3, &d_pos));
    TSC_TRY(h.out(out, size_t(n_poses) * ft.n_total * 3, &d_out));
    TSC_TRY(tsc_transform_batch_dev(c, d_frags, frag_off, n_atoms, n_conf, n_mols, d_ci, d_rot, d_pos, n_poses, d_out));
    return h.finish();
    TSC_API_GUARD_END
}


static int make_clash_args(int64_t n_poses, int n_atoms, const int32_t *ids, int n_ids, double thresh, int64_t max_clashes,
                           ClashArgs *a) {
    TSC_REQUIRE(n_poses >= 0 && n_atoms > 0, "bad sizes");
    TSC_REQUIRE(n_ids == 0 || n_ids == 2 || n_ids == 3, "ids must have 0 (None), 2 or 3 entries, got %d", n_ids);
    memset(a, 0, sizeof(*a));
    a->n_poses = n_poses;
    a->n = n_atoms;
    a->max_clashes = max_clashes;
    if (n_ids == 0) {
        a->self_mode = 1;
        a->first_row = 0;
        a->n_mols = 1;
        a->sq_bound = clash_sq_bound(0.5);
        for (int m = 1; m <= MAX_MOLS; ++m) a->atom_off[m] = n_atoms;
    } else {
        TSC_REQUIRE(ids != nullptr, "ids is null");
        int off = 0;
        for (int m = 0; m < n_ids; ++m) {
            a->atom_off[m] = off;
            TSC_REQUIRE(ids[m] >= 0, "negative fragment length");
            off += ids[m];
        }
        TSC_REQUIRE(off - ids[n_ids - 1] <= n_atoms, "fragment lengths exceed the atom count");
        for (int m = n_ids; m <= MAX_MOLS; ++m) a->atom_off[m] = n_atoms;
        a->n_mols = n_ids;
        a->first_row = a->atom_off[1];
        a->sq_bound = clash_sq_bound(thresh);
    }
    int rows = std::max(1, n_atoms - a->first_row);
    a->lp = std::min(64, std::max(4, pow2_ceil(rows)));
    return 0;
}

template <bool FUSED, bool SELF, bool MINMODE>
static int launch_clash_impl(tsc_ctx *c, const ClashArgs &a, const double *coords, const double *frags, const FragTable &ft,
                             const int32_t *conf_idx, const double *rot, const double *pos, uint8_t *mask, int32_t *counts) {
    const int ppw = 64 / a.lp;
    size_t lds = size_t(4) * clash_lds_per_wave(a.n, a.lp, MINMODE);
    TSC_REQUIRE(lds <= 160 * 1024, "pose too large for the LDS staging of the clash kernel (%d atoms)", a.n);
    int64_t waves = ceil_div<int64_t>(a.n_poses, ppw);
    int blocks = grid_for(waves, 4, 256 * 32);
    TSC_TRY(lds_attribute(&k_clash<FUSED, SELF, MINMODE>, lds));
    hipLaunchKernelGGL((k_clash<FUSED, SELF, MINMODE>), dim3(blocks), dim3(256), lds, c->stream, a, coords, frags, ft, conf_idx, rot, pos, mask, counts);
    TSC_HIP(hipGetLastError());
    return 0;
}

template <bool FUSED>
static int launch_clash(tsc_ctx *c, const ClashArgs &a, const double *coords, const double *frags, const FragTable &ft,
                        const int32_t *conf_idx, const double *rot, const double *pos, uint8_t *mask, int32_t *counts) {
    if (a.n_poses == 0) return 0;
    if (a.self_mode) return launch_clash_impl<FUSED, true, false>(c, a, coords, frags, ft, conf_idx, rot, pos, mask, counts);
    const bool minmode = !counts && a.max_clashes == 0 && c->opt.clash_fp32 != 0 && 4 * clash_lds_per_wave(a.n, a.lp, true) <= 160 * 1024;
    if (minmode && FUSED && c->opt.clash_lanes != 0 && a.n_mols == 2 && ft.n_mols == 2 && a.atom_off[1] == ft.atom_off[1] && a.n == ft.n_total &&
        std::min(ft.n_atoms[0], ft.n_atoms[1]) >= 1 && std::min(ft.n_atoms[0], ft.n_atoms[1]) <= 32) {
        const int mA = ft.n_atoms[0] <= ft.n_atoms[1] ? 0 : 1, mB = 1 - mA, na2 = (ft.n_atoms[mA] + 1) / 2;
        const dim3 grid(unsigned(grid_for(ceil_div<int64_t>(a.n_poses, 64), 4, 256 * 32)));
#define TSC_LAUNCH_CLASH_LANES(N)                                                                                                          \
    hipLaunchKernelGGL(k_clash_lanes<N>, grid, dim3(256), 0, c->stream, a.n_poses, frags, ft, mA, mB, conf_idx, rot, pos, a.sq_bound, mask)
        if (na2 <= 4) TSC_LAUNCH_CLASH_LANES(4);
        else if (na2 <= 8) TSC_LAUNCH_CLASH_LANES(8);
        else if (na2 <= 12) TSC_LAUNCH_CLASH_LANES(12);
        else if (na2 <= 13) TSC_LAUNCH_CLASH_LANES(13);
        else TSC_LAUNCH_CLASH_LANES(16);
#undef TSC_LAUNCH_CLASH_LANES
        TSC_HIP(hipGetLastError());
        return 0;
    }
    if (minmode && FUSED && c->opt.clash_lanes != 0 && (a.n_mols == 2 || a.n_mols == 3) && ft.n_mols == a.n_mols && a.n == ft.n_total &&
        a.atom_off[1] == ft.atom_off[1] && (a.n_mols == 2 || a.atom_off[2] == ft.atom_off[2])) {
        auto cost = [&](int na2) {
            int64_t w = 0;
            const int n_pairs = a.n_mols == 2 ? 1 : 3;
            for (int pr = 0; pr < n_pairs; ++pr) {
                const int mA = a.n_mols == 2 ? 1 : (pr == 0 ? 1 : (pr == 1 ? 2 : 0)), mB = a.n_mols == 2 ? 0 : (pr == 0 ? 0 : (pr == 1 ? 1 : 2));
                const int64_t tiles = ceil_div(ft.n_atoms[mA], 2 * na2);
                w += tiles * ft.n_atoms[mB] * (2 * na2 + 4);
            }
            return w;
        };
        int best = 12;
        for (int na2 : {16, 18})
            if (cost(na2) < cost(best)) best = na2;
        const dim3 grid(unsigned(grid_for(ceil_div<int64_t>(a.n_poses, CLM_POSES), 1, 256 * 32)));
#define TSC_LAUNCH_CLASH_MULTI(N)                                                                                                          \
    hipLaunchKernelGGL(k_clash_lanes_multi<N>, grid, dim3(256), 0, c->stream, a.n_poses, frags, ft, conf_idx, rot, pos, a.sq_bound, mask)
        if (best == 12) TSC_LAUNCH_CLASH_MULTI(12);
        else if (best == 16) TSC_LAUNCH_CLASH_MULTI(16);
        else TSC_LAUNCH_CLASH_MULTI(18);
#undef TSC_LAUNCH_CLASH_MULTI
        TSC_HIP(hipGetLastError());
        return 0;
    }
    if (minmode) return launch_clash_impl<FUSED, false, true>(c, a, coords, frags, ft, conf_idx, rot, pos, mask, counts);
    return launch_clash_impl<FUSED, false, false>(c, a, coords, frags, ft, conf_idx, rot, pos, mask, counts);
}

extern "C" __attribute__((visibility("default"))) int tsc_clash_mask_dev(tsc_ctx *c, const double *coords, int64_t n_poses, int n_atoms, const int32_t *ids, int n_ids,
                                  double thresh, int64_t max_clashes, uint8_t *mask, int32_t *counts) {
    TSC_API_GUARD_BEGIN
    TSC_REQUIRE(c && coords && mask, "tsc_clash_mask_dev: null argument");
    ClashArgs a;
    TSC_TRY(make_clash_args(n_poses, n_atoms, ids, n_ids, thresh, max_clashes, &a));
    DeviceGuard guard(c->device);
    FragTable ft;
    memset(&ft, 0, sizeof(ft));
    return launch_clash<false>(c, a, coords, nullptr, ft, nullptr, nullptr, nullptr, mask, counts);
    TSC_API_GUARD_END
}

extern "C" __attribute__((visibility("default"))) int tsc_clash_mask(tsc_ctx *c, const double *coords, int64_t n_poses, int n_atoms, const int32_t *ids, int n_ids,
                              double thresh, int64_t max_clashes, uint8_t *mask, int32_t *counts) {
    TSC_API_GUARD_BEGIN
    TSC_REQUIRE(c && coords && mask, "tsc_clash_mask: null argument");
    ClashArgs a;
    TSC_TRY(make_clash_args(n_poses, n_atoms, ids, n_ids, thresh, max_clashes, &a));
    if (n_poses == 0) return 0;
    HostCall h(c);
    double *d_coords;
    uint8_t *d_mask;
    int32_t *d_counts;
    TSC_TRY(h.in(coords, size_t(n_poses) * n_atoms * 3, &d_coords));
    TSC_TRY(h.out(mask, size_t(n_poses), &d_mask));
    TSC_TRY(h.out(counts, size_t(n_poses), &d_counts));
    TSC_TRY(tsc_clash_mask_dev(c, d_coords, n_poses, n_atoms, ids, n_ids, thresh, max_clashes, d_mask, d_counts));
    return h.finish();
    TSC_API_GUARD_END
}

extern "C" __attribute__((visibility("default"))) int tsc_embed_clash_mask_dev(tsc_ctx *c, const double *frags, const int64_t *frag_off, const int32_t *n_atoms,
                                        const int32_t *n_conf, int n_mols, const int32_t *conf_idx, const double *rot,
                                        const double *pos, int64_t n_poses, double thresh, int64_t max_clashes, uint8_t *mask,
                                        int32_t *counts) {
    TSC_API_GUARD_BEGIN
    TSC_REQUIRE(c && frags && conf_idx && rot && pos && mask, "tsc_embed_clash_mask_dev: null argument");
    TSC_REQUIRE(n_mols == 2 || n_mols == 3, "the fused embed+clash path needs 2 or 3 fragments, got %d", n_mols);
    FragTable ft;
    TSC_TRY(make_frag_table(frag_off, n_atoms, n_conf, n_mols, &ft));
    ClashArgs a;
    TSC_TRY(make_clash_args(n_poses, ft.n_total, n_atoms, n_mols, thresh, max_clashes, &a));
    DeviceGuard guard(c->device);
    return launch_clash<true>(c, a, nullptr, frags, ft, conf_idx, rot, pos, mask, counts);
    TSC_API_GUARD_END
}

extern "C" __attribute__((visibility("default"))) int tsc_all_dists(tsc_ctx *c, const double *A, int na, const double *B, int nb, double *out) {
    TSC_API_GUARD_BEGIN
    TSC_REQUIRE(c && A && B && out && na >= 0 && nb >= 0, "tsc_all_dists: bad argument");
    if (na == 0 || nb == 0) return 0;
    HostCall h(c);
    double *dA, *dB, *dO;
    TSC_TRY(h.in(A, size_t(na) * 3, &dA));
    TSC_TRY(h.in(B, size_t(nb) * 3, &dB));
    TSC_TRY(h.out(out, size_t(na) * nb, &dO));
    hipLaunchKernelGGL(k_all_dists, dim3(grid_for(int64_t(na) * nb, 256)), dim3(256), 0, c->stream, dA, na, dB, nb, dO);
    TSC_HIP(hipGetLastError());
    return h.finish();
    TSC_API_GUARD_END
}



extern "C" __attribute__((visibility("default"))) int tsc_compact_rows_dev(tsc_ctx *c, const void *src, const uint8_t *mask, int64_t n_rows, int64_t row_bytes, void *dst,
                                    int64_t *n_kept_host) {
    TSC_API_GUARD_BEGIN
    TSC_REQUIRE(c && src && mask && dst, "tsc_compact_rows_dev: null argument");
    TSC_REQUIRE(n_rows >= 0 && n_rows < INT32_MAX && row_bytes > 0 && row_bytes % 8 == 0 && row_bytes / 8 < INT32_MAX, "bad sizes");
    if (n_rows == 0) {
        if (n_kept_host) *n_kept_host = 0;
        return 0;
    }
    DeviceGuard guard(c->device);
    Scratch s(c);
    int32_t *bsum, *act, *total;
    TSC_TRY(s.get(scan_bsum_count(n_rows), &bsum));
    TSC_TRY(s.get(size_t(n_rows), &act));
    TSC_TRY(s.get(1, &total));
    TSC_TRY(scan_mask(c->stream, mask, n_rows, bsum, nullptr, act, nullptr, total));
    int32_t kept = 0;
    TSC_TRY(read_i32(c, total, &kept));
    TSC_TRY(launch_gather_rows(c->stream, src, act, kept, int(row_bytes / 8), nullptr, int(row_bytes / 8), dst));
    if (n_kept_host) *n_kept_host = kept;
    return 0;
    TSC_API_GUARD_END
}

extern "C" __attribute__((visibility("default"))) int tsc_gather_heavy_dev(tsc_ctx *c, const double *coords, const uint8_t *mask, int64_t n_poses, int n_atoms,
                                    const int32_t *heavy_idx, int n_heavy, double *heavy_out, int64_t *n_kept_host) {
    TSC_API_GUARD_BEGIN
    TSC_REQUIRE(c && coords && heavy_idx && heavy_out, "tsc_gather_heavy_dev: null argument");
    TSC_REQUIRE(n_poses >= 0 && n_poses < INT32_MAX && n_atoms > 0 && n_heavy > 0 && n_heavy <= n_atoms, "bad sizes");
    if (n_poses == 0) {
        if (n_kept_host) *n_kept_host = 0;
        return 0;
    }
    DeviceGuard guard(c->device);
    Scratch s(c);
    std::vector<int32_t> sel(size_t(n_heavy) * 3);
    for (int a = 0; a < n_heavy; ++a) {
        TSC_REQUIRE(heavy_idx[a] >= 0 && heavy_idx[a] < n_atoms, "heavy_idx[%d] out of range", a);
        for (int k = 0; k < 3; ++k) sel[size_t(a) * 3 + k] = heavy_idx[a] * 3 + k;
    }
    int32_t *d_sel, *act = nullptr;
    TSC_TRY(upload(c, s, sel.data(), sel.size(), &d_sel));
    int32_t kept = int32_t(n_poses);
    if (mask) {
        int32_t *bsum, *total;
        TSC_TRY(s.get(scan_bsum_count(n_poses), &bsum));
        TSC_TRY(s.get(size_t(n_poses), &act));
        TSC_TRY(s.get(1, &total));
        TSC_TRY(scan_mask(c->stream, mask, n_poses, bsum, nullptr, act, nullptr, total));
        TSC_TRY(read_i32(c, total, &kept));
    } else {
        TSC_HIP(hipStreamSynchronize(c->stream));
    }
    TSC_TRY(launch_gather_rows(c->stream, coords, act, kept, n_atoms * 3, d_sel, n_heavy * 3, heavy_out));
    if (!mask) TSC_HIP(hipStreamSynchronize(c->stream));
    if (n_kept_host) *n_kept_host = kept;
    return 0;
    TSC_API_GUARD_END
}
```

### tscode_amd/csrc/embed_clash.hpp

```cpp
#pragma once
#include "common.hpp"

namespace tsc {

constexpr int MAX_MOLS = 8;

struct FragTable {
    int n_mols;
    int n_total;
    long long frag_off[MAX_MOLS];
    int n_atoms[MAX_MOLS];
    int n_conf[MAX_MOLS];
    int atom_off[MAX_MOLS + 1];
};

__device__ inline int frag_of_atom(const FragTable &ft, int a) {
    int m = 0;
#pragma unroll
    for (int k = 1; k < MAX_MOLS; ++k)
        if (k < ft.n_mols && a >= ft.atom_off[k]) m = k;
    return m;
}

__device__ inline void embed_atom(const double *__restrict__ frags, const FragTable &ft, const int32_t *__restrict__ conf_idx,
                                  const double *__restrict__ rot, const double *__restrict__ pos, int64_t s, int a, double out[3]) {
    int m = frag_of_atom(ft, a);
    int64_t sm = s * ft.n_mols + m;
    const double *X = frags + ft.frag_off[m] + (int64_t(conf_idx[sm]) * ft.n_atoms[m] + (a - ft.atom_off[m])) * 3;
    const double *R = rot + sm * 9;
    const double *t = pos + sm * 3;
    double x0 = X[0], x1 = X[1], x2 = X[2];
#pragma unroll
    for (int i = 0; i < 3; ++i) out[i] = R[3 * i] * x0 + R[3 * i + 1] * x1 + R[3 * i + 2] * x2 + t[i];
}

__device__ inline void embed_atom_staged(const double *__restrict__ frags, const FragTable &ft, const double *sR, const double *sT, const int *sC,
                                         int local_pose, int a, double out[3]) {
    const int m = frag_of_atom(ft, a), l = local_pose * ft.n_mols + m;
    const double *X = frags + ft.frag_off[m] + (int64_t(sC[l]) * ft.n_atoms[m] + (a - ft.atom_off[m])) * 3;
    const double *R = sR + l * 9, *t = sT + l * 3;
    const double x0 = X[0], x1 = X[1], x2 = X[2];
#pragma unroll
    for (int i = 0; i < 3; ++i) out[i] = R[3 * i] * x0 + R[3 * i + 1] * x1 + R[3 * i + 2] * x2 + t[i];
}

constexpr int TR_POSES = 32;
__host__ __device__ inline size_t transform_lds_bytes(int n_mols) { return size_t(TR_POSES) * n_mols * (12 * sizeof(double) + sizeof(int)) + TR_POSES * sizeof(int64_t); }

struct ClashArgs {
    int64_t n_poses;
    int n;
    int first_row;
    int self_mode;
    int lp;
    int n_mols;
    int atom_off[MAX_MOLS + 1];
    double sq_bound;
    long long max_clashes;
};

inline double clash_sq_bound(double thresh) {
    if (!(thresh > 0)) return 0.0;
    double x = thresh * thresh;
    while (std::sqrt(x) >= thresh) x = std::nextafter(x, 0.0);
    while (std::sqrt(x) < thresh) x = std::nextafter(x, INFINITY);
    return x;
}

typedef float clash_f32x2 __attribute__((ext_vector_type(2)));

__host__ __device__ inline size_t clash_lds_per_wave(int n, int lp, bool minmode) {
    const int ppw = 64 / lp, npad = (n + 1) & ~1;
    return size_t(ppw) * n * 3 * sizeof(double) + (minmode ? size_t(ppw) * 3 * npad * sizeof(float) : 0);
}

__device__ inline bool fp32_min_band(double x0, double cmax, float *lo_out, float *hi_out) {
    constexpr double U = 5.9604644775390625e-08;
    const double e = 4.0 * U * cmax * (1.0 + U);
    const double M = 1.01 * (8.0 * U * x0 + (2.0 * 1.7320508075688774 * e * sqrt(x0) + 3.0 * e * e) * (1.0 + 4.0 * U));
    float lo = float(x0 - M), hi = float(x0 + M);
    if (double(lo) > x0 - M) lo = __uint_as_float(__float_as_uint(lo) - 1u);
    if (double(hi) < x0 + M) hi = __uint_as_float(__float_as_uint(hi) + 1u);
    *lo_out = lo, *hi_out = hi;
    return cmax < 1.0e15 && x0 - M > 0.0;
}

inline int pow2_ceil(int v) {
    int p = 1;
    while (p < v) p <<= 1;
    return p;
}

}
```

### tscode_amd/csrc/embed_transform.hpp

```cpp
#pragma once
#include "embed_clash.hpp"

namespace tsc {

inline __global__ __launch_bounds__(256) void k_transform(const double *__restrict__ frags, FragTable ft,
                                                    const int32_t *__restrict__ conf_idx, const double *__restrict__ rot,
                                                    const double *__restrict__ pos, const int32_t *__restrict__ idx,
                                                    int64_t n_out, double *__restrict__ out,
                                                    const int32_t *__restrict__ heavy_slot, int n_heavy,
                                                    double *__restrict__ heavy_out, const int32_t *__restrict__ n_out_dev,
                                                    double *__restrict__ zero_me = nullptr, int n_zero = 0) {
    extern __shared__ __attribute__((aligned(16))) double s_tr[];
    const int n = ft.n_total, nm = ft.n_mols, tid = threadIdx.x;
    for (int e = blockIdx.x * 256 + tid; e < n_zero; e += gridDim.x * 256) zero_me[e] = 0.0;
    if (n_out_dev) n_out = *n_out_dev;
    int64_t *sP = reinterpret_cast<int64_t *>(s_tr);
    double *sR = s_tr + TR_POSES, *sT = sR + TR_POSES * nm * 9;
    int *sC = reinterpret_cast<int *>(sT + TR_POSES * nm * 3);
    for (int64_t r0 = int64_t(blockIdx.x) * TR_POSES; r0 < n_out; r0 += int64_t(gridDim.x) * TR_POSES) {
        const int np = int(min<int64_t>(TR_POSES, n_out - r0));
        if (tid < np) sP[tid] = idx ? int64_t(idx[r0 + tid]) : r0 + tid;
        __syncthreads();
        for (int q = tid; q < np * nm * 9; q += 256) {
            const int row = q / (nm * 9), w = q - row * nm * 9;
            sR[q] = rot[sP[row] * nm * 9 + w];
        }
        for (int q = tid; q < np * nm * 3; q += 256) {
            const int row = q / (nm * 3), w = q - row * nm * 3;
            sT[q] = pos[sP[row] * nm * 3 + w];
        }
        for (int q = tid; q < np * nm; q += 256) {
            const int row = q / nm, w = q - row * nm;
            sC[q] = conf_idx[sP[row] * nm + w];
        }
        __syncthreads();
        for (int e = tid; e < np * n; e += 256) {
            const int row = e / n, a = e - row * n;
            const int64_t r = r0 + row;
            double v[3];
            embed_atom_staged(frags, ft, sR, sT, sC, row, a, v);
            if (out) {
                double *o = out + (r * n + a) * 3;
                o[0] = v[0];
                o[1] = v[1];
                o[2] = v[2];
            }
            if (heavy_out) {
                const int hs = heavy_slot[a];
                if (hs >= 0) {
                    double *h = heavy_out + (r * n_heavy + hs) * 3;
                    h[0] = v[0];
                    h[1] = v[1];
                    h[2] = v[2];
                }
            }
        }
        __syncthreads();
    }
}

}
```

### tscode_amd/csrc/pipeline.hip

```cpp
#include "host.hpp"
#include "embed_transform.hpp"
#include "scan_kernels.hpp"
#include "prune_api.hpp"
#include "descriptor_basis.hpp"
#include "describe.hpp"
#include "sample_moments.hpp"


static int heavy_slot_table(tsc_ctx *c, const FragTable &ft, const int32_t *heavy_idx, int n_heavy, int32_t **d_slot) {
    std::vector<int32_t> slot(size_t(ft.n_total), -1);
    for (int a = 0; a < n_heavy; ++a) {
        TSC_REQUIRE(heavy_idx[a] >= 0 && heavy_idx[a] < ft.n_total && (a == 0 || heavy_idx[a] > heavy_idx[a - 1]),
                    "heavy_idx must be strictly increasing atom indices");
        slot[size_t(heavy_idx[a])] = a;
    }
    if (!(c->slot_dev && c->slot_host == slot)) {
        if (c->slot_dev) c->release(c->slot_dev);
        c->slot_dev = nullptr;
        void *q = nullptr;
        TSC_TRY(c->alloc(slot.size() * sizeof(int32_t), &q));
        c->slot_dev = static_cast<int32_t *>(q);
        c->slot_host = slot;
        TSC_HIP(hipMemcpyAsync(c->slot_dev, c->slot_host.data(), slot.size() * sizeof(int32_t), hipMemcpyHostToDevice, c->stream));
    }
    *d_slot = c->slot_dev;
    return 0;
}

static int basis_sample_table(tsc_ctx *c, int64_t n_poses, int *n_samples_out) {
    const int n_samples = int(std::min<int64_t>(n_poses, DESC_SAMPLE));
    const int64_t stride = std::max<int64_t>(1, n_poses / n_samples);
    if (!(c->sample_dev && int(c->sample_host.size()) == n_samples && c->sample_host.back() == int32_t(stride * (n_samples - 1)))) {
        if (c->sample_dev) c->release(c->sample_dev);
        c->sample_dev = nullptr;
        c->sample_host.resize(size_t(n_samples));
        for (int i = 0; i < n_samples; ++i) c->sample_host[size_t(i)] = int32_t(stride * i);
        void *q = nullptr;
        TSC_TRY(c->alloc(size_t(n_samples) * sizeof(int32_t), &q));
        c->sample_dev = static_cast<int32_t *>(q);
        TSC_HIP(hipMemcpyAsync(c->sample_dev, c->sample_host.data(), size_t(n_samples) * sizeof(int32_t), hipMemcpyHostToDevice, c->stream));
    }
    *n_samples_out = n_samples;
    return 0;
}

struct BasisFork {
    int n_samples = 0;
    double *sample = nullptr, *moments = nullptr, *basis = nullptr;
};
static int basis_fork_begin(tsc_ctx *c, int64_t n_poses, int n_heavy, BasisFork *bf) {
    *bf = BasisFork();
    if (!(c->opt.early_basis && c->opt.prune_algo != ALGO_TILE)) return 0;
    TSC_TRY(basis_sample_table(c, n_poses, &bf->n_samples));
    const size_t need = size_t(bf->n_samples) * n_heavy * 3 + moment_doubles(n_heavy) + basis_doubles(n_heavy);
    if (!(c->eb_block && c->eb_h == n_heavy && c->eb_samples == bf->n_samples)) {
        TSC_HIP(hipStreamSynchronize(c->basis_stream));
        if (c->eb_block) c->release(c->eb_block);
        c->eb_block = nullptr;
        void *q = nullptr;
        TSC_TRY(c->alloc(need * sizeof(double), &q));
        c->eb_block = static_cast<double *>(q), c->eb_h = n_heavy, c->eb_samples = bf->n_samples;
    }
    bf->sample = c->eb_block, bf->moments = bf->sample + size_t(bf->n_samples) * n_heavy * 3, bf->basis = bf->moments + moment_doubles(n_heavy);
    TSC_HIP(hipEventRecord(c->ev_fork, c->stream));
    return 0;
}
static int basis_fork_launch(tsc_ctx *c, const BasisFork &bf, Scratch &s, const double *frags, const FragTable &ft, const int32_t *conf_idx, const double *rot,
                             const double *pos, const int32_t *d_slot, int n_heavy) {
    if (!bf.basis) return 0;
    TSC_HIP(hipStreamWaitEvent(c->basis_stream, c->ev_fork, 0));
    hipLaunchKernelGGL(k_transform, dim3(grid_for(bf.n_samples, TR_POSES, 256 * 64)), dim3(256), transform_lds_bytes(ft.n_mols), c->basis_stream, frags, ft, conf_idx,
                       rot, pos, (const int32_t *)c->sample_dev, int64_t(bf.n_samples), (double *)nullptr, (const int32_t *)d_slot, n_heavy, bf.sample,
                       (const int32_t *)nullptr, bf.moments, int(moment_doubles(n_heavy)));
    TSC_TRY(build_basis(c, c->basis_stream, s, bf.sample, n_heavy, bf.n_samples, 1, bf.basis, nullptr, bf.moments));
    TSC_HIP(hipEventRecord(c->ev_join, c->basis_stream));
    c->eb_valid = true;
    return 0;
}
const double *pending_basis(const tsc_ctx *c, int h) {
    return (c->eb_valid && c->eb_h == h && c->opt.prune_algo != ALGO_TILE) ? c->eb_block + size_t(c->eb_samples) * h * 3 + moment_doubles(h) : nullptr;
}

extern "C" __attribute__((visibility("default"))) int tsc_basis_from_poses_dev(tsc_ctx *c, const double *frags, const int64_t *frag_off, const int32_t *n_atoms,
                                                                               const int32_t *n_conf, int n_mols, const int32_t *conf_idx, const double *rot,
                                                                               const double *pos, int64_t n_poses, const int32_t *heavy_idx, int n_heavy) {
    TSC_API_GUARD_BEGIN
    TSC_REQUIRE(c && frags && conf_idx && rot && pos && heavy_idx, "tsc_basis_from_poses_dev: null argument");
    TSC_REQUIRE(n_poses > 0 && n_poses < INT32_MAX, "bad n_poses");
    FragTable ft;
    TSC_TRY(make_frag_table(frag_off, n_atoms, n_conf, n_mols, &ft));
    TSC_REQUIRE(n_heavy > 0 && n_heavy <= ft.n_total, "bad n_heavy");
    DeviceGuard guard(c->device);
    Scratch s(c);
    int32_t *d_slot;
    TSC_TRY(heavy_slot_table(c, ft, heavy_idx, n_heavy, &d_slot));
    BasisFork bf;
    TSC_TRY(basis_fork_begin(c, n_poses, n_heavy, &bf));
    return basis_fork_launch(c, bf, s, frags, ft, conf_idx, rot, pos, d_slot, n_heavy);
    TSC_API_GUARD_END
}

extern "C" __attribute__((visibility("default"))) int tsc_embed_masked_dev(tsc_ctx *c, const double *frags, const int64_t *frag_off, const int32_t *n_atoms,
                                                                           const int32_t *n_conf, int n_mols, const int32_t *conf_idx, const double *rot,
                                                                           const double *pos, int64_t n_poses, const uint8_t *mask, const int32_t *heavy_idx,
                                                                           int n_heavy, double *structures, double *heavy, int64_t *n_sel_host) {
    TSC_API_GUARD_BEGIN
    TSC_REQUIRE(c && frags && conf_idx && rot && pos && heavy_idx && mask && (structures || heavy), "tsc_embed_masked_dev: null argument");
    TSC_REQUIRE(n_poses >= 0 && n_poses < INT32_MAX, "bad n_poses");
    if (n_sel_host) *n_sel_host = 0;
    if (n_poses == 0) return 0;
    FragTable ft;
    TSC_TRY(make_frag_table(frag_off, n_atoms, n_conf, n_mols, &ft));
    TSC_REQUIRE(n_heavy > 0 && n_heavy <= ft.n_total, "bad n_heavy");
    DeviceGuard guard(c->device);
    hipStream_t st = c->stream;
    Scratch s(c);
    int32_t *d_slot, *bsum, *act, *total;
    TSC_TRY(heavy_slot_table(c, ft, heavy_idx, n_heavy, &d_slot));
    TSC_TRY(s.get(scan_bsum_count(n_poses), &bsum));
    TSC_TRY(s.get(size_t(n_poses), &act));
    TSC_TRY(s.get(1, &total));
    TSC_TRY(scan_mask(st, mask, n_poses, bsum, nullptr, act, nullptr, total));
    if (n_sel_host) TSC_TRY(read_i32_begin(c, total));
    const double *basis = heavy ? pending_basis(c, n_heavy) : nullptr;
    c->xd_valid = false;
    if (basis && c->opt.fuse_descriptors && transform_describe_lds_bytes(ft.n_mols, n_heavy) <= 64 * 1024) {
        if (!(c->xd_D && c->xd_cap >= n_poses)) {
            if (c->xd_borrowers > 0)
                return fail(TSC_ERR_STATE, "tsc_embed_masked_dev: %d live prune run(s) still read the descriptor buffers of an earlier call, which %lld poses "
                                           "would outgrow: destroy them first (tsc_prune_destroy)", c->xd_borrowers, (long long)n_poses);
            for (void *q : {static_cast<void *>(c->xd_D), static_cast<void *>(c->xd_G), static_cast<void *>(c->xd_dmax)})
                if (q) c->release(q);
            c->xd_D = nullptr, c->xd_G = nullptr, c->xd_dmax = nullptr, c->xd_cap = 0;
            void *q = nullptr;
            TSC_TRY(c->alloc(size_t(n_poses) * DW * sizeof(float), &q));
            c->xd_D = static_cast<float *>(q);
            TSC_TRY(c->alloc(size_t(n_poses) * sizeof(double), &q));
            c->xd_G = static_cast<double *>(q);
            TSC_TRY(c->alloc(4 * sizeof(unsigned), &q));
            c->xd_dmax = static_cast<unsigned *>(q);
            c->xd_cap = n_poses;
        }
        const int nf0 = n_features(n_heavy, 0), nf1 = n_features(n_heavy, 1);
        float *h32 = nullptr;
        if (want_heavy32(c->opt, double(n_poses) * n_heavy * 24.0)) {
            const int64_t need = n_poses * heavy32_pitch(n_heavy);
            if (c->xd_h32_cap < need) {
                if (c->xd_borrowers > 0)
                    return fail(TSC_ERR_STATE, "tsc_embed_masked_dev: %d live prune run(s) still read the float32 copy of an earlier call: destroy them first",
                                c->xd_borrowers);
                if (c->xd_heavy32) c->release(c->xd_heavy32);
                c->xd_heavy32 = nullptr, c->xd_h32_cap = 0;
                void *q = nullptr;
                TSC_TRY(c->alloc(size_t(need) * sizeof(float), &q));
                c->xd_heavy32 = static_cast<float *>(q), c->xd_h32_cap = need;
            }
            h32 = c->xd_heavy32;
        }
        TSC_HIP(hipMemsetAsync(c->xd_dmax, 0, sizeof(unsigned), st));
        TSC_HIP(hipStreamWaitEvent(st, c->ev_join, 0));
        hipLaunchKernelGGL(k_transform_describe, dim3(grid_for(n_poses, TR_POSES, 256 * 64)), dim3(256), transform_describe_lds_bytes(ft.n_mols, n_heavy), st,
                           frags, ft, conf_idx, rot, pos, (const int32_t *)act, structures, (const int32_t *)d_slot, n_heavy, heavy, (const int32_t *)total,
                           nf0, nf1, basis, (const double *)(basis + size_t(KD) * (nf0 + nf1)), c->xd_D, c->xd_G, c->xd_dmax, h32);
        c->xd_valid = true, c->xd_h = n_heavy, c->xd_heavy = heavy, c->xd_h32_valid = h32 != nullptr;
        c->eb_valid = false;
    } else {
        hipLaunchKernelGGL(k_transform, dim3(grid_for(n_poses, TR_POSES, 256 * 64)), dim3(256), transform_lds_bytes(ft.n_mols), st, frags, ft, conf_idx, rot, pos,
                           (const int32_t *)act, int64_t(0), structures, (const int32_t *)d_slot, heavy ? n_heavy : 0, heavy, (const int32_t *)total);
    }
    TSC_HIP(hipGetLastError());
    if (n_sel_host) {
        int32_t n_sel = 0;
        TSC_TRY(read_i32_finish(c, &n_sel));
        *n_sel_host = n_sel;
    }
    return 0;
    TSC_API_GUARD_END
}

extern "C" __attribute__((visibility("default"))) int tsc_embed_clash_compact_dev(tsc_ctx *c, const double *frags, const int64_t *frag_off, const int32_t *n_atoms,
                                                                                  const int32_t *n_conf, int n_mols, const int32_t *conf_idx, const double *rot,
                                                                                  const double *pos, int64_t n_poses, const int32_t *heavy_idx, int n_heavy,
                                                                                  double clash_thresh, int64_t max_clashes, uint8_t *clash_mask,
                                                                                  double *structures, double *heavy, int64_t *n_pass_host) {
    TSC_API_GUARD_BEGIN
    TSC_REQUIRE(c && frags && conf_idx && rot && pos && heavy_idx && clash_mask && heavy && n_pass_host, "tsc_embed_clash_compact_dev: null argument");
    TSC_REQUIRE(n_poses >= 0 && n_poses < INT32_MAX, "bad n_poses");
    *n_pass_host = 0;
    if (n_poses == 0) return 0;
    FragTable ft;
    TSC_TRY(make_frag_table(frag_off, n_atoms, n_conf, n_mols, &ft));
    TSC_REQUIRE(n_heavy > 0 && n_heavy <= ft.n_total, "bad n_heavy");
    DeviceGuard guard(c->device);
    hipStream_t st = c->stream;
    Scratch s(c);
    int32_t *d_slot, *bsum, *act, *total;
    TSC_TRY(heavy_slot_table(c, ft, heavy_idx, n_heavy, &d_slot));
    TSC_TRY(s.get(scan_bsum_count(n_poses), &bsum));
    TSC_TRY(s.get(size_t(n_poses), &act));
    TSC_TRY(s.get(1, &total));
    BasisFork bf;
    TSC_TRY(basis_fork_begin(c, n_poses, n_heavy, &bf));
    TSC_TRY(tsc_embed_clash_mask_dev(c, frags, frag_off, n_atoms, n_conf, n_mols, conf_idx, rot, pos, n_poses, clash_thresh, max_clashes, clash_mask, nullptr));
    TSC_TRY(basis_fork_launch(c, bf, s, frags, ft, conf_idx, rot, pos, d_slot, n_heavy));
    TSC_TRY(scan_mask(st, clash_mask, n_poses, bsum, nullptr, act, nullptr, total));
    TSC_TRY(read_i32_begin(c, total));
    hipLaunchKernelGGL(k_transform, dim3(grid_for(n_poses, TR_POSES, 256 * 64)), dim3(256), transform_lds_bytes(ft.n_mols), st, frags, ft, conf_idx, rot, pos, (const int32_t *)act,
                       int64_t(0), structures, (const int32_t *)d_slot, n_heavy, heavy, (const int32_t *)total);
    TSC_HIP(hipGetLastError());
    int32_t n_pass = 0;
    TSC_TRY(read_i32_finish(c, &n_pass));
    *n_pass_host = n_pass;
    return 0;
    TSC_API_GUARD_END
}

extern "C" __attribute__((visibility("default"))) int tsc_pipeline_dev(tsc_ctx *c, const double *frags, const int64_t *frag_off, const int32_t *n_atoms, const int32_t *n_conf,
                                int n_mols, const int32_t *conf_idx, const double *rot, const double *pos, int64_t n_poses,
                                const int32_t *heavy_idx, int n_heavy, double clash_thresh, int64_t max_clashes, double rmsd_thr, int mode,
                                uint8_t *clash_mask, double *structures, uint8_t *keep_mask, uint8_t *keep_mask_host, int64_t *n_pass_host,
                                int64_t *n_keep_host, tsc_pass_stats *stats, int *n_passes, float *timings_ms) {
    TSC_API_GUARD_BEGIN
    TSC_REQUIRE(c && frags && conf_idx && rot && pos && heavy_idx && clash_mask && structures && keep_mask, "tsc_pipeline_dev: null argument");
    TSC_REQUIRE(n_poses > 0 && n_poses < INT32_MAX, "bad n_poses");
    FragTable ft;
    TSC_TRY(make_frag_table(frag_off, n_atoms, n_conf, n_mols, &ft));
    TSC_REQUIRE(n_heavy > 0 && n_heavy <= ft.n_total, "bad n_heavy");
    DeviceGuard guard(c->device);
    hipStream_t st = c->stream;
    Scratch s(c);
    const bool timed = timings_ms && c->opt.pass_timing >= 2;
    hipEvent_t ev[4] = {nullptr, nullptr, nullptr, nullptr};
    struct EvGuard {
        tsc_ctx *c;
        hipEvent_t *e;
        ~EvGuard() {
            for (int i = 0; i < 4; ++i)
                if (e[i]) c->event_pool.push_back(e[i]);
        }
    } evg{c, ev};
    if (timed)
        for (auto &e : ev) TSC_TRY(get_event(c, &e));
    int32_t *d_slot, *bsum, *act, *total;
    double *d_heavy;
    TSC_TRY(heavy_slot_table(c, ft, heavy_idx, n_heavy, &d_slot));
    TSC_TRY(s.get(scan_bsum_count(n_poses), &bsum));
    TSC_TRY(s.get(size_t(n_poses), &act));
    TSC_TRY(s.get(1, &total));
    if (timed) TSC_HIP(hipEventRecord(ev[0], st));
    double *d_basis = nullptr;
    ExternalDescriptors ext;
    struct BasisJoin {
        tsc_ctx *c;
        bool pending;
        ~BasisJoin() {
            if (pending) (void)hipStreamSynchronize(c->basis_stream);
        }
    } basis_join{c, false};
    int n_samples = 0;
    double *d_sample = nullptr, *d_moments = nullptr;
    bool fused_sample = false;
    if (c->opt.early_basis && c->opt.prune_algo != ALGO_TILE) {
        TSC_TRY(basis_sample_table(c, n_poses, &n_samples));
        TSC_TRY(s.get(size_t(n_samples) * n_heavy * 3, &d_sample));
        TSC_TRY(s.get(basis_doubles(n_heavy), &d_basis));
        if (c->opt.fuse_descriptors && transform_describe_lds_bytes(ft.n_mols, n_heavy) <= 64 * 1024) {
            TSC_TRY(s.get(size_t(n_poses) * DW, &ext.D));
            TSC_TRY(s.get(size_t(n_poses), &ext.G));
            TSC_TRY(s.get(4, &ext.dmax_bits));
            if (want_heavy32(c->opt, double(n_poses) * n_heavy * 24.0))
                TSC_TRY(s.get(size_t(n_poses) * heavy32_pitch(n_heavy), &ext.heavy32));
        }
        fused_sample = !c->opt.deterministic_basis && sample_moments_lds_bytes(ft.n_mols, n_heavy) <= 64 * 1024;
        if (fused_sample) {
            const size_t a = size_t(n_features(n_heavy, 0) + 1), b = size_t(n_features(n_heavy, 1) + 1), need = a * a + b * b;
            if (c->mom_cap < need) {
                if (c->mom_acc) c->release(c->mom_acc);
                c->mom_acc = nullptr, c->mom_cap = 0;
                void *q = nullptr;
                TSC_TRY(c->alloc(need * sizeof(double), &q));
                c->mom_acc = static_cast<double *>(q), c->mom_cap = need, c->mom_clean = false;
            }
            if (!c->mom_clean) TSC_HIP(hipMemsetAsync(c->mom_acc, 0, c->mom_cap * sizeof(double), st));
        } else {
            TSC_TRY(s.get(moment_doubles(n_heavy), &d_moments));
        }
        TSC_HIP(hipEventRecord(c->ev_fork, st));
    }
    auto enqueue_basis_chain = [&]() -> int {
        TSC_HIP(hipStreamWaitEvent(c->basis_stream, c->ev_fork, 0));
        basis_join.pending = true;
        double *spread_host = reinterpret_cast<double *>(static_cast<char *>(c->pinned) + PINNED_SPREAD_OFFSET);
        spread_host[0] = spread_host[1] = __builtin_inf();
        if (fused_sample) {
            const int nf0 = n_features(n_heavy, 0), nf1 = n_features(n_heavy, 1);
            c->mom_clean = false;
            hipLaunchKernelGGL(k_sample_moments, dim3(ceil_div(ceil_div(n_samples, TR_POSES), SM_CHUNKS), NFAM), dim3(256), sample_moments_lds_bytes(ft.n_mols, n_heavy), c->basis_stream,
                               frags, ft, conf_idx, rot, pos, (const int32_t *)c->sample_dev, n_samples, (const int32_t *)d_slot, n_heavy, nf0, nf1, c->mom_acc,
                               c->mom_acc + size_t(nf0 + 1) * (nf0 + 1));
            hipLaunchKernelGGL(k_descriptor_basis, dim3(NFAM), dim3(64), 0, c->basis_stream, (const double *)c->mom_acc,
                               (const double *)(c->mom_acc + size_t(nf0 + 1) * (nf0 + 1)), nf0, nf1, n_samples, d_basis, d_basis + size_t(KD) * (nf0 + nf1),
                               ext.dmax_bits, spread_host, 1);
            TSC_HIP(hipGetLastError());
            c->mom_clean = true;
        } else {
            hipLaunchKernelGGL(k_transform, dim3(grid_for(n_samples, TR_POSES, 256 * 64)), dim3(256), transform_lds_bytes(ft.n_mols), c->basis_stream, frags, ft,
                               conf_idx, rot, pos, (const int32_t *)c->sample_dev, int64_t(n_samples), (double *)nullptr, (const int32_t *)d_slot, n_heavy, d_sample,
                               (const int32_t *)nullptr, d_moments, int(moment_doubles(n_heavy)));
            TSC_TRY(build_basis(c, c->basis_stream, s, d_sample, n_heavy, n_samples, 1, d_basis, ext.dmax_bits, d_moments, spread_host));
        }
        TSC_HIP(hipEventRecord(c->ev_join, c->basis_stream));
        return 0;
    };
    if (d_basis && !c->opt.clash_first) TSC_TRY(enqueue_basis_chain());
    TSC_TRY(tsc_embed_clash_mask_dev(c, frags, frag_off, n_atoms, n_conf, n_mols, conf_idx, rot, pos, n_poses, clash_thresh, max_clashes,
                                     clash_mask, nullptr));
    if (timed) TSC_HIP(hipEventRecord(ev[1], st));
    if (d_basis && c->opt.clash_first) TSC_TRY(enqueue_basis_chain());
    volatile int32_t *count_host = reinterpret_cast<volatile int32_t *>(static_cast<char *>(c->pinned) + PINNED_COUNT_OFFSET);
    *count_host = -1;
    TSC_TRY(scan_mask(st, clash_mask, n_poses, bsum, nullptr, act, nullptr, total, nullptr, false, const_cast<int32_t *>(count_host)));
    TSC_TRY(s.get(size_t(n_poses) * n_heavy * 3, &d_heavy));
    if (ext.D) {
        const int nf0 = n_features(n_heavy, 0), nf1 = n_features(n_heavy, 1);
        TSC_HIP(hipStreamWaitEvent(st, c->ev_join, 0));
        hipLaunchKernelGGL(k_transform_describe, dim3(grid_for(n_poses, TR_POSES, 256 * 64)), dim3(256), transform_describe_lds_bytes(ft.n_mols, n_heavy), st,
                           frags, ft, conf_idx, rot, pos, (const int32_t *)act, structures, (const int32_t *)d_slot, n_heavy, d_heavy, (const int32_t *)total,
                           nf0, nf1, (const double *)d_basis, (const double *)(d_basis + size_t(KD) * (nf0 + nf1)), ext.D, ext.G, ext.dmax_bits, ext.heavy32);
    } else {
        hipLaunchKernelGGL(k_transform, dim3(grid_for(n_poses, TR_POSES, 256 * 64)), dim3(256), transform_lds_bytes(ft.n_mols), st, frags, ft, conf_idx, rot, pos,
                           (const int32_t *)act, int64_t(0), structures, (const int32_t *)d_slot, n_heavy, d_heavy, (const int32_t *)total);
    }
    TSC_HIP(hipGetLastError());
    int32_t n_pass = -1;
    {
        const auto t_look = std::chrono::steady_clock::now();
        for (unsigned spins = 0; (n_pass = *count_host) < 0; ++spins) {
            __builtin_ia32_pause();
            if ((spins & 0xffffu) == 0xffffu && std::chrono::steady_clock::now() - t_look > std::chrono::seconds(5)) {
                TSC_TRY(read_i32(c, total, &n_pass));
                break;
            }
        }
    }
    if (n_pass_host) *n_pass_host = n_pass;
    int64_t n_keep = 0;
    int np = 0;
    if (d_basis) TSC_HIP(hipStreamWaitEvent(st, c->ev_join, 0));
    int force_algo = -1;
    if (d_basis && c->opt.prune_algo == ALGO_AUTO && mode == 1 && n_heavy <= MAX_HP) {
        TSC_HIP(hipEventSynchronize(c->ev_join));
        const volatile double *sh = reinterpret_cast<const volatile double *>(static_cast<const char *>(c->pinned) + PINNED_SPREAD_OFFSET);
        const double spread[NFAM] = {sh[0], sh[1]};
        if (screen_is_useless(spread, n_heavy, rmsd_thr)) force_algo = ALGO_TILE;
    }
    const bool sieve_run = force_algo != ALGO_TILE;
    if (n_pass > 0) {
        if (timed) TSC_HIP(hipEventRecord(ev[2], st));
        TSC_TRY(prune_run(c, d_heavy, n_pass, n_heavy, rmsd_thr, mode, keep_mask, keep_mask_host, stats, &np, sieve_run ? d_basis : nullptr,
                          (sieve_run && ext.D) ? &ext : nullptr, force_algo));
        for (int i = 0; i < np; ++i) n_keep = stats ? stats[i].n_active_after : 0;
        if (!stats) {
            TSC_TRY(scan_mask(st, keep_mask, n_pass, bsum, nullptr, nullptr, nullptr, total));
            int32_t t = 0;
            TSC_TRY(read_i32(c, total, &t));
            n_keep = t;
        }
    } else if (timed) {
        TSC_HIP(hipEventRecord(ev[2], st));
    }
    if (timed) {
        TSC_HIP(hipEventRecord(ev[3], st));
        TSC_HIP(hipEventSynchronize(ev[3]));
    } else {
        TSC_HIP(hipStreamSynchronize(st));
    }
    if (n_passes) *n_passes = np;
    if (n_keep_host) *n_keep_host = n_keep;
    if (timings_ms && !timed) timings_ms[0] = timings_ms[1] = timings_ms[2] = timings_ms[3] = 0.0f;
    if (timed) {
        TSC_HIP(hipEventElapsedTime(&timings_ms[0], ev[0], ev[1]));
        TSC_HIP(hipEventElapsedTime(&timings_ms[1], ev[1], ev[2]));
        TSC_HIP(hipEventElapsedTime(&timings_ms[2], ev[2], ev[3]));
        TSC_HIP(hipEventElapsedTime(&timings_ms[3], ev[0], ev[3]));
    }
    return 0;
    TSC_API_GUARD_END
}
```

### tscode_amd/csrc/sample_moments.hpp

```cpp
#pragma once
#include "descriptor.hpp"
#include "embed_clash.hpp"

namespace tsc {

constexpr int SM_CHUNKS = 1;
__host__ __device__ inline size_t sample_moments_lds_bytes(int n_mols, int h) {
    return (transform_lds_bytes(n_mols) + 15) / 16 * 16 + size_t(TR_POSES) * (size_t(h) * 3 + size_t(h) + 1) * sizeof(double);
}
inline __global__ __launch_bounds__(256) void k_sample_moments(const double *__restrict__ frags, FragTable ft, const int32_t *__restrict__ conf_idx,
                                                        const double *__restrict__ rot, const double *__restrict__ pos,
                                                        const int32_t *__restrict__ sample_idx, int n_samples, const int32_t *__restrict__ heavy_slot,
                                                        int h, int nf0, int nf1, double *__restrict__ M0, double *__restrict__ M1) {
    extern __shared__ __attribute__((aligned(16))) unsigned char s_sm_raw[];
    const int fam = blockIdx.y, nf = fam == 0 ? nf0 : nf1;
    if (nf == 0) return;
    const int n = ft.n_total, nm = ft.n_mols, tid = threadIdx.x, m = nf + 1;
    double *s_tr = reinterpret_cast<double *>(s_sm_raw);
    int64_t *sP = reinterpret_cast<int64_t *>(s_tr);
    double *sR = s_tr + TR_POSES, *sT = sR + TR_POSES * nm * 9;
    int *sC = reinterpret_cast<int *>(sT + TR_POSES * nm * 3);
    double *s_x = reinterpret_cast<double *>(s_sm_raw + (transform_lds_bytes(nm) + 15) / 16 * 16);
    double *s_n = s_x + size_t(TR_POSES) * h * 3;
    double *__restrict__ Mf = fam == 0 ? M0 : M1;
    const int n_chunks = (n_samples + TR_POSES - 1) / TR_POSES;
    constexpr int ACC = 8;
    const bool in_regs = m * m <= 256 * ACC;
    double acc[ACC];
#pragma unroll
    for (int u = 0; u < ACC; ++u) acc[u] = 0.0;
    for (int ch = blockIdx.x * SM_CHUNKS; ch < min(n_chunks, (int(blockIdx.x) + 1) * SM_CHUNKS); ++ch) {
        const int s0 = ch * TR_POSES, ns = min(TR_POSES, n_samples - s0);
        if (tid < ns) sP[tid] = int64_t(sample_idx[s0 + tid]);
        __syncthreads();
        for (int q = tid; q < ns * nm * 9; q += 256) {
            const int row = q / (nm * 9), w = q - row * nm * 9;
            sR[q] = rot[sP[row] * nm * 9 + w];
        }
        for (int q = tid; q < ns * nm * 3; q += 256) {
            const int row = q / (nm * 3), w = q - row * nm * 3;
            sT[q] = pos[sP[row] * nm * 3 + w];
        }
        for (int q = tid; q < ns * nm; q += 256) {
            const int row = q / nm, w = q - row * nm;
            sC[q] = conf_idx[sP[row] * nm + w];
        }
        __syncthreads();
        for (int e = tid; e < ns * n; e += 256) {
            const int row = e / n, a = e - row * n;
            const int hs = heavy_slot[a];
            if (hs < 0) continue;
            double v[3];
            embed_atom_staged(frags, ft, sR, sT, sC, row, a, v);
            double *o = s_x + (size_t(row) * h + hs) * 3;
            o[0] = v[0], o[1] = v[1], o[2] = v[2];
        }
        __syncthreads();
        for (int e = tid; e < ns * m; e += 256) {
            const int sm = e / m, a = e - sm * m;
            s_n[sm * m + a] = (a < nf) ? feature(s_x + size_t(sm) * h * 3, h, fam, a) : 1.0;
        }
        __syncthreads();
        if (in_regs) {
#pragma unroll
            for (int u = 0; u < ACC; ++u) {
                const int e = tid + 256 * u;
                if (e < m * m) {
                    const int a = e / m, b = e - a * m;
                    if (b >= a) {
                        double t = 0.0;
                        for (int sm = 0; sm < ns; ++sm) t += s_n[sm * m + a] * s_n[sm * m + b];
                        acc[u] += t;
                    }
                }
            }
        } else {
            for (int e = tid; e < m * m; e += 256) {
                const int a = e / m, b = e - a * m;
                if (b < a) continue;
                double t = 0.0;
                for (int sm = 0; sm < ns; ++sm) t += s_n[sm * m + a] * s_n[sm * m + b];
                atomicAdd(&Mf[e], t);
            }
        }
        __syncthreads();
    }
    if (in_regs) {
#pragma unroll
        for (int u = 0; u < ACC; ++u) {
            const int e = tid + 256 * u;
            if (e < m * m && e % m >= e / m) atomicAdd(&Mf[e], acc[u]);
        }
    }
}

}
```

Before: 159.8 million.

## Stage per-atom fragment table in LDS and batch pose-parameter loads in embed kernels

Adds a per-block LDS table of per-atom fragment base, stride and heavy slot, so the embed loops stop running frag_of_atom and reading heavy_slot from global memory for every atom. Pose parameter staging is batched into register loads followed by one waitcnt, and the next pose index and Q/bias are prefetched before the loop. The embed loop is templated to batch several atom loads per thread, and a lighter LDS-only barrier is used before the describe step. LDS use per block grows with n_total, which may lower occupancy or push the fused describe path over its 64KB limit.

```diff
diff --git a/tscode_amd/csrc/adjacent.hip b/tscode_amd/csrc/adjacent.hip
--- a/tscode_amd/csrc/adjacent.hip
+++ b/tscode_amd/csrc/adjacent.hip
@@ -596,7 +596,7 @@
         double *d_structs;
         TSC_TRY(s.get(size_t(n_pass) * n * 3, &d_structs));
         TSC_TRY(s.get(size_t(n_pass), &d_acc));
-        hipLaunchKernelGGL(k_transform, dim3(grid_for(n_pass, TR_POSES, 256 * 64)), dim3(256), transform_lds_bytes(ft.n_mols), st, d_frags, ft, d_ci, d_rot, d_pos,
+        hipLaunchKernelGGL(k_transform, dim3(grid_for(n_pass, TR_POSES, 256 * 64)), dim3(256), transform_lds_bytes(ft.n_mols, ft.n_total), st, d_frags, ft, d_ci, d_rot, d_pos,
                            (const int32_t *)act, int64_t(n_pass), d_structs, (const int32_t *)nullptr, 0, (double *)nullptr, (const int32_t *)nullptr);
         TSC_HIP(hipGetLastError());
         f->structs = d_structs;
@@ -1118,7 +1118,7 @@
     }
     double *d_out;
     TSC_TRY(s.get(size_t(rows) * n * 3, &d_out));
-    hipLaunchKernelGGL(k_transform, dim3(grid_for(rows, TR_POSES, 256 * 64)), dim3(256), transform_lds_bytes(r->ft.n_mols), c->stream, (const double *)r->frags, r->ft,
+    hipLaunchKernelGGL(k_transform, dim3(grid_for(rows, TR_POSES, 256 * 64)), dim3(256), transform_lds_bytes(r->ft.n_mols, r->ft.n_total), c->stream, (const double *)r->frags, r->ft,
                        (const int32_t *)r->ci, (const double *)r->rot, (const double *)r->pos, (const int32_t *)act, rows, d_out, (const int32_t *)nullptr, 0,
                        (double *)nullptr, (const int32_t *)nullptr);
     TSC_HIP(hipGetLastError());
diff --git a/tscode_amd/csrc/describe.hpp b/tscode_amd/csrc/describe.hpp
--- a/tscode_amd/csrc/describe.hpp
+++ b/tscode_amd/csrc/describe.hpp
@@ -81,49 +81,50 @@
     describe_from_lds(s_q, s_x, pitch, h, nf0, nf1, bias, ns, S, i0, D, G, dmax_bits);
 }
 
+constexpr int TD_BATCH = 1;
 inline __global__ __launch_bounds__(256) void k_transform_describe(const double *__restrict__ frags, FragTable ft, const int32_t *__restrict__ conf_idx,
                                                              const double *__restrict__ rot, const double *__restrict__ pos,
-                                                             const int32_t *__restrict__ idx, double *__restrict__ out,
+                                                             const int32_t *__restrict__ idx, int64_t idx_len, double *__restrict__ out,
                                                              const int32_t *__restrict__ heavy_slot, int n_heavy, double *__restrict__ heavy_out,
                                                              const int32_t *__restrict__ n_out_dev, int nf0, int nf1, const double *__restrict__ Q,
                                                              const double *__restrict__ bias, float *__restrict__ D, double *__restrict__ G,
                                                              unsigned *__restrict__ dmax_bits, float *__restrict__ heavy32_out = nullptr) {
     extern __shared__ __attribute__((aligned(16))) double s_tr[];
     const int n = ft.n_total, nm = ft.n_mols, tid = threadIdx.x, pitch = (n_heavy * 3) | 1;
-    const int pitch32 = heavy32_pitch(n_heavy), pad32 = pitch32 - 3 * n_heavy;
+    const int pitch32 = heavy32_pitch(n_heavy), pad32 = pitch32 - 3 * n_heavy, nq = KD * (nf0 + nf1);
+    int64_t r0 = int64_t(blockIdx.x) * TR_POSES;
+    int32_t pose = idx[min<int64_t>(r0 + tid, idx_len - 1)];
+    const int slot = tid < n ? heavy_slot[tid] : -1;
+    const double bias_k = tid < DW ? bias[tid] : 0.0;
+    double qv[2];
+#pragma unroll
+    for (int j = 0; j < 2; ++j) qv[j] = tid + 256 * j < nq ? Q[tid + 256 * j] : 0.0;
     const int64_t n_out = *n_out_dev;
     int64_t *sP = reinterpret_cast<int64_t *>(s_tr);
     double *sR = s_tr + TR_POSES, *sT = sR + TR_POSES * nm * 9;
     int *sC = reinterpret_cast<int *>(sT + TR_POSES * nm * 3);
-    double *s_q = s_tr + (transform_lds_bytes(nm) + 15) / 16 * 2, *s_x = s_q + KD * (nf0 + nf1);
-    for (int e = tid; e < KD * (nf0 + nf1); e += 256) s_q[e] = Q[e];
-    for (int64_t r0 = int64_t(blockIdx.x) * TR_POSES; r0 < n_out; r0 += int64_t(gridDim.x) * TR_POSES) {
+    AtomEntry *tab = reinterpret_cast<AtomEntry *>(s_tr + (pose_params_lds_bytes(nm) + 15) / 16 * 2);
+    double *s_bias = s_tr + transform_lds_bytes(nm, n) / 8, *s_q = s_bias + DW, *s_x = s_q + nq;
+    build_atom_table(tab, ft, heavy_slot, slot);
+    if (tid < DW) s_bias[tid] = bias_k;
+#pragma unroll
+    for (int j = 0; j < 2; ++j)
+        if (tid + 256 * j < nq) s_q[tid + 256 * j] = qv[j];
+    for (int e = tid + 512; e < nq; e += 256) s_q[e] = Q[e];
+    wait_vector_loads();
+    for (bool first = true; r0 < n_out; first = false, r0 += int64_t(gridDim.x) * TR_POSES) {
         const int np = int(min<int64_t>(TR_POSES, n_out - r0));
-        if (tid < np) sP[tid] = int64_t(idx[r0 + tid]);
+        if (!first) pose = idx[min<int64_t>(r0 + tid, idx_len - 1)];
+        if (tid < np) sP[tid] = int64_t(pose);
         __syncthreads();
-        for (int q = tid; q < np * nm * 9; q += 256) {
-            const int row = q / (nm * 9), w = q - row * nm * 9;
-            sR[q] = rot[sP[row] * nm * 9 + w];
-        }
-        for (int q = tid; q < np * nm * 3; q += 256) {
-            const int row = q / (nm * 3), w = q - row * nm * 3;
-            sT[q] = pos[sP[row] * nm * 3 + w];
-        }
-        for (int q = tid; q < np * nm; q += 256) {
-            const int row = q / nm, w = q - row * nm;
-            sC[q] = conf_idx[sP[row] * nm + w];
-        }
+        stage_pose_params(sP, sR, sT, sC, conf_idx, rot, pos, np, nm);
         __syncthreads();
-        for (int e = tid; e < np * n; e += 256) {
-            const int row = e / n, a = e - row * n;
+        embed_tile<TD_BATCH, false>(frags, tab, sR, sT, sC, np, n, nm, [&](int row, int a, int hs, const double *v) {
             const int64_t r = r0 + row;
-            double v[3];
-            embed_atom_staged(frags, ft, sR, sT, sC, row, a, v);
             if (out) {
                 double *o = out + (r * n + a) * 3;
                 o[0] = v[0], o[1] = v[1], o[2] = v[2];
             }
-            const int hs = heavy_slot[a];
             if (hs >= 0) {
                 double *hv = heavy_out + (r * n_heavy + hs) * 3, *x = s_x + row * pitch + hs * 3;
                 hv[0] = x[0] = v[0], hv[1] = x[1] = v[1], hv[2] = x[2] = v[2];
@@ -132,17 +133,17 @@
                     hf[0] = float(v[0]), hf[1] = float(v[1]), hf[2] = float(v[2]);
                 }
             }
-        }
+        });
         if (heavy32_out)
             for (int e = tid; e < np * pad32; e += 256) heavy32_out[(r0 + e / pad32) * pitch32 + 3 * n_heavy + e % pad32] = 0.0f;
-        __syncthreads();
-        describe_from_lds(s_q, s_x, pitch, n_heavy, nf0, nf1, bias, np, TR_POSES, r0, D, G, dmax_bits);
+        lds_barrier();
+        describe_from_lds(s_q, s_x, pitch, n_heavy, nf0, nf1, s_bias, np, TR_POSES, r0, D, G, dmax_bits);
         __syncthreads();
     }
 }
 
-inline size_t transform_describe_lds_bytes(int n_mols, int h) {
-    return (transform_lds_bytes(n_mols) + 15) / 16 * 16 + (size_t(KD) * (n_features(h, 0) + n_features(h, 1)) + size_t(TR_POSES) * ((h * 3) | 1)) * sizeof(double);
+inline size_t transform_describe_lds_bytes(int n_mols, int n_total, int h) {
+    return transform_lds_bytes(n_mols, n_total) + (size_t(DW) + size_t(KD) * (n_features(h, 0) + n_features(h, 1)) + size_t(TR_POSES) * ((h * 3) | 1)) * sizeof(double);
 }
 
 }
diff --git a/tscode_amd/csrc/embed.hip b/tscode_amd/csrc/embed.hip
--- a/tscode_amd/csrc/embed.hip
+++ b/tscode_amd/csrc/embed.hip
@@ -16,7 +16,7 @@
     TSC_TRY(make_frag_table(frag_off, n_atoms, n_conf, n_mols, &ft));
     if (n_poses == 0) return 0;
     DeviceGuard guard(c->device);
-    hipLaunchKernelGGL(k_transform, dim3(grid_for(n_poses, TR_POSES, 256 * 64)), dim3(256), transform_lds_bytes(ft.n_mols), c->stream, frags, ft, conf_idx, rot,
+    hipLaunchKernelGGL(k_transform, dim3(grid_for(n_poses, TR_POSES, 256 * 64)), dim3(256), transform_lds_bytes(ft.n_mols, ft.n_total), c->stream, frags, ft, conf_idx, rot,
                        pos, (const int32_t *)nullptr, n_poses, out, (const int32_t *)nullptr, 0, (double *)nullptr, (const int32_t *)nullptr);
     TSC_HIP(hipGetLastError());
     return 0;
diff --git a/tscode_amd/csrc/embed_clash.hpp b/tscode_amd/csrc/embed_clash.hpp
--- a/tscode_amd/csrc/embed_clash.hpp
+++ b/tscode_amd/csrc/embed_clash.hpp
@@ -34,18 +34,117 @@
     for (int i = 0; i < 3; ++i) out[i] = R[3 * i] * x0 + R[3 * i + 1] * x1 + R[3 * i + 2] * x2 + t[i];
 }
 
-__device__ inline void embed_atom_staged(const double *__restrict__ frags, const FragTable &ft, const double *sR, const double *sT, const int *sC,
-                                         int local_pose, int a, double out[3]) {
-    const int m = frag_of_atom(ft, a), l = local_pose * ft.n_mols + m;
-    const double *X = frags + ft.frag_off[m] + (int64_t(sC[l]) * ft.n_atoms[m] + (a - ft.atom_off[m])) * 3;
-    const double *R = sR + l * 9, *t = sT + l * 3;
-    const double x0 = X[0], x1 = X[1], x2 = X[2];
-#pragma unroll
-    for (int i = 0; i < 3; ++i) out[i] = R[3 * i] * x0 + R[3 * i + 1] * x1 + R[3 * i + 2] * x2 + t[i];
+__device__ inline void lds_barrier() {
+    __builtin_amdgcn_fence(__ATOMIC_RELEASE, "workgroup", "local");
+    __builtin_amdgcn_s_barrier();
+    __builtin_amdgcn_fence(__ATOMIC_ACQUIRE, "workgroup", "local");
 }
 
+__device__ inline void wait_vector_loads() { __builtin_amdgcn_s_waitcnt(0x0F70); }
+
 constexpr int TR_POSES = 32;
-__host__ __device__ inline size_t transform_lds_bytes(int n_mols) { return size_t(TR_POSES) * n_mols * (12 * sizeof(double) + sizeof(int)) + TR_POSES * sizeof(int64_t); }
+__host__ __device__ inline size_t pose_params_lds_bytes(int n_mols) { return size_t(TR_POSES) * n_mols * (12 * sizeof(double) + sizeof(int)) + TR_POSES * sizeof(int64_t); }
+
+struct __attribute__((aligned(16))) AtomEntry {
+    long long base;
+    int stride;
+    int key;
+};
+__host__ __device__ inline size_t transform_lds_bytes(int n_mols, int n_total) {
+    return (pose_params_lds_bytes(n_mols) + 15) / 16 * 16 + size_t(n_total) * sizeof(AtomEntry);
+}
+
+__device__ inline AtomEntry atom_entry(const FragTable &ft, int a, int heavy_slot) {
+    int m = 0, first = 0, count = ft.n_atoms[0];
+    long long off = ft.frag_off[0];
+#pragma unroll
+    for (int k = 1; k < MAX_MOLS; ++k)
+        if (k < ft.n_mols && a >= ft.atom_off[k]) m = k, first = ft.atom_off[k], count = ft.n_atoms[k], off = ft.frag_off[k];
+    return AtomEntry{off + (long long)(a - first) * 3, count * 3, m | (heavy_slot + 1) << 3};
+}
+
+__device__ inline void build_atom_table(AtomEntry *tab, const FragTable &ft, const int32_t *__restrict__ heavy_slot, int first_slot) {
+    for (int a = threadIdx.x; a < ft.n_total; a += 256) {
+        const int hs = a < 256 ? first_slot : (heavy_slot ? heavy_slot[a] : -1);
+        tab[a] = atom_entry(ft, a, hs);
+    }
+}
+
+__device__ inline void stage_pose_params(const int64_t *sP, double *sR, double *sT, int *sC, const int32_t *__restrict__ conf_idx,
+                                         const double *__restrict__ rot, const double *__restrict__ pos, int np, int nm) {
+    constexpr int BR = 4, BT = 2;
+    const int tid = threadIdx.x, cr = np * nm * 9, ct = np * nm * 3, cc = np * nm;
+    for (int b = 0; b * 256 * BR < cr; ++b) {
+        double r[BR], t[BT];
+        int ci = 0;
+#pragma unroll
+        for (int j = 0; j < BR; ++j) {
+            const int q = tid + 256 * (b * BR + j), row = q / (nm * 9);
+            r[j] = q < cr ? rot[sP[row] * nm * 9 + (q - row * nm * 9)] : 0.0;
+        }
+#pragma unroll
+        for (int j = 0; j < BT; ++j) {
+            const int q = tid + 256 * (b * BT + j), row = q / (nm * 3);
+            t[j] = q < ct ? pos[sP[row] * nm * 3 + (q - row * nm * 3)] : 0.0;
+        }
+        {
+            const int q = min(tid + 256 * b, cc - 1), row = q / nm;
+            ci = conf_idx[sP[row] * nm + (q - row * nm)];
+        }
+        wait_vector_loads();
+#pragma unroll
+        for (int j = 0; j < BR; ++j) {
+            const int q = tid + 256 * (b * BR + j);
+            if (q < cr) sR[q] = r[j];
+        }
+#pragma unroll
+        for (int j = 0; j < BT; ++j) {
+            const int q = tid + 256 * (b * BT + j);
+            if (q < ct) sT[q] = t[j];
+        }
+        if (tid + 256 * b < cc) sC[tid + 256 * b] = ci;
+    }
+}
+
+template <int B, bool HEAVY_ONLY, typename Sink>
+__device__ inline void embed_tile(const double *__restrict__ frags, const AtomEntry *tab, const double *sR, const double *sT, const int *sC, int np, int n,
+                                  int nm, Sink sink) {
+    const int total = np * n, dq = 256 / n, dr = 256 - dq * n;
+    int row = int(threadIdx.x) / n, a = int(threadIdx.x) - row * n;
+    for (int base = threadIdx.x; base < total; base += 256 * B) {
+        double x[B][3];
+        int lk[B];
+        const int row0 = row, a0 = a;
+#pragma unroll
+        for (int j = 0; j < B; ++j) {
+            const AtomEntry t = tab[a];
+            const bool todo = base + 256 * j < total && (!HEAVY_ONLY || (t.key >> 3) > 0);
+            const int l = todo ? row * nm + (t.key & 7) : 0;
+            lk[j] = todo ? l | (t.key >> 3) << 8 : -1;
+            const double *X = todo ? frags + t.base + int64_t(sC[l]) * t.stride : frags;
+            x[j][0] = X[0], x[j][1] = X[1], x[j][2] = X[2];
+            row += dq, a += dr;
+            if (a >= n) a -= n, ++row;
+        }
+        wait_vector_loads();
+        int row1 = row0, a1 = a0;
+        asm volatile("" : "+v"(row1), "+v"(a1));
+#pragma unroll
+        for (int j = 0; j < B; ++j) {
+            if (lk[j] >= 0) {
+                const int l = lk[j] & 255;
+                const double *R = sR + l * 9, *t = sT + l * 3;
+                const double x0 = x[j][0], x1 = x[j][1], x2 = x[j][2];
+                double v[3];
+#pragma unroll
+                for (int i = 0; i < 3; ++i) v[i] = R[3 * i] * x0 + R[3 * i + 1] * x1 + R[3 * i + 2] * x2 + t[i];
+                sink(row1, a1, (lk[j] >> 8) - 1, v);
+            }
+            row1 += dq, a1 += dr;
+            if (a1 >= n) a1 -= n, ++row1;
+        }
+    }
+}
 
 struct ClashArgs {
     int64_t n_poses;
diff --git a/tscode_amd/csrc/embed_transform.hpp b/tscode_amd/csrc/embed_transform.hpp
--- a/tscode_amd/csrc/embed_transform.hpp
+++ b/tscode_amd/csrc/embed_transform.hpp
@@ -13,48 +13,39 @@
     extern __shared__ __attribute__((aligned(16))) double s_tr[];
     const int n = ft.n_total, nm = ft.n_mols, tid = threadIdx.x;
     for (int e = blockIdx.x * 256 + tid; e < n_zero; e += gridDim.x * 256) zero_me[e] = 0.0;
+    const int64_t idx_len = n_out;
+    int64_t r0 = int64_t(blockIdx.x) * TR_POSES;
+    int32_t pose = (idx && idx_len > 0) ? idx[min<int64_t>(r0 + tid, idx_len - 1)] : 0;
+    const int slot = (heavy_out && tid < n) ? heavy_slot[tid] : -1;
     if (n_out_dev) n_out = *n_out_dev;
     int64_t *sP = reinterpret_cast<int64_t *>(s_tr);
     double *sR = s_tr + TR_POSES, *sT = sR + TR_POSES * nm * 9;
     int *sC = reinterpret_cast<int *>(sT + TR_POSES * nm * 3);
-    for (int64_t r0 = int64_t(blockIdx.x) * TR_POSES; r0 < n_out; r0 += int64_t(gridDim.x) * TR_POSES) {
+    AtomEntry *tab = reinterpret_cast<AtomEntry *>(s_tr + (pose_params_lds_bytes(nm) + 15) / 16 * 2);
+    build_atom_table(tab, ft, heavy_out ? heavy_slot : nullptr, slot);
+    wait_vector_loads();
+    for (bool first = true; r0 < n_out; first = false, r0 += int64_t(gridDim.x) * TR_POSES) {
         const int np = int(min<int64_t>(TR_POSES, n_out - r0));
-        if (tid < np) sP[tid] = idx ? int64_t(idx[r0 + tid]) : r0 + tid;
+        if (idx && !first) pose = idx[min<int64_t>(r0 + tid, idx_len - 1)];
+        if (tid < np) sP[tid] = idx ? int64_t(pose) : r0 + tid;
         __syncthreads();
-        for (int q = tid; q < np * nm * 9; q += 256) {
-            const int row = q / (nm * 9), w = q - row * nm * 9;
-            sR[q] = rot[sP[row] * nm * 9 + w];
-        }
-        for (int q = tid; q < np * nm * 3; q += 256) {
-            const int row = q / (nm * 3), w = q - row * nm * 3;
-            sT[q] = pos[sP[row] * nm * 3 + w];
-        }
-        for (int q = tid; q < np * nm; q += 256) {
-            const int row = q / nm, w = q - row * nm;
-            sC[q] = conf_idx[sP[row] * nm + w];
-        }
+        stage_pose_params(sP, sR, sT, sC, conf_idx, rot, pos, np, nm);
         __syncthreads();
-        for (int e = tid; e < np * n; e += 256) {
-            const int row = e / n, a = e - row * n;
+        embed_tile<1, false>(frags, tab, sR, sT, sC, np, n, nm, [&](int row, int a, int hs, const double *v) {
             const int64_t r = r0 + row;
-            double v[3];
-            embed_atom_staged(frags, ft, sR, sT, sC, row, a, v);
             if (out) {
                 double *o = out + (r * n + a) * 3;
                 o[0] = v[0];
                 o[1] = v[1];
                 o[2] = v[2];
             }
-            if (heavy_out) {
-                const int hs = heavy_slot[a];
-                if (hs >= 0) {
-                    double *h = heavy_out + (r * n_heavy + hs) * 3;
-                    h[0] = v[0];
-                    h[1] = v[1];
-                    h[2] = v[2];
-                }
+            if (hs >= 0) {
+                double *h = heavy_out + (r * n_heavy + hs) * 3;
+                h[0] = v[0];
+                h[1] = v[1];
+                h[2] = v[2];
             }
-        }
+        });
         __syncthreads();
     }
 }
diff --git a/tscode_amd/csrc/pipeline.hip b/tscode_amd/csrc/pipeline.hip
--- a/tscode_amd/csrc/pipeline.hip
+++ b/tscode_amd/csrc/pipeline.hip
@@ -69,7 +69,7 @@
                              const double *pos, const int32_t *d_slot, int n_heavy) {
     if (!bf.basis) return 0;
     TSC_HIP(hipStreamWaitEvent(c->basis_stream, c->ev_fork, 0));
-    hipLaunchKernelGGL(k_transform, dim3(grid_for(bf.n_samples, TR_POSES, 256 * 64)), dim3(256), transform_lds_bytes(ft.n_mols), c->basis_stream, frags, ft, conf_idx,
+    hipLaunchKernelGGL(k_transform, dim3(grid_for(bf.n_samples, TR_POSES, 256 * 64)), dim3(256), transform_lds_bytes(ft.n_mols, ft.n_total), c->basis_stream, frags, ft, conf_idx,
                        rot, pos, (const int32_t *)c->sample_dev, int64_t(bf.n_samples), (double *)nullptr, (const int32_t *)d_slot, n_heavy, bf.sample,
                        (const int32_t *)nullptr, bf.moments, int(moment_doubles(n_heavy)));
     TSC_TRY(build_basis(c, c->basis_stream, s, bf.sample, n_heavy, bf.n_samples, 1, bf.basis, nullptr, bf.moments));
@@ -124,7 +124,7 @@
     if (n_sel_host) TSC_TRY(read_i32_begin(c, total));
     const double *basis = heavy ? pending_basis(c, n_heavy) : nullptr;
     c->xd_valid = false;
-    if (basis && c->opt.fuse_descriptors && transform_describe_lds_bytes(ft.n_mols, n_heavy) <= 64 * 1024) {
+    if (basis && c->opt.fuse_descriptors && transform_describe_lds_bytes(ft.n_mols, ft.n_total, n_heavy) <= 64 * 1024) {
         if (!(c->xd_D && c->xd_cap >= n_poses)) {
             if (c->xd_borrowers > 0)
                 return fail(TSC_ERR_STATE, "tsc_embed_masked_dev: %d live prune run(s) still read the descriptor buffers of an earlier call, which %lld poses "
@@ -159,14 +159,14 @@
         }
         TSC_HIP(hipMemsetAsync(c->xd_dmax, 0, sizeof(unsigned), st));
         TSC_HIP(hipStreamWaitEvent(st, c->ev_join, 0));
-        hipLaunchKernelGGL(k_transform_describe, dim3(grid_for(n_poses, TR_POSES, 256 * 64)), dim3(256), transform_describe_lds_bytes(ft.n_mols, n_heavy), st,
-                           frags, ft, conf_idx, rot, pos, (const int32_t *)act, structures, (const int32_t *)d_slot, n_heavy, heavy, (const int32_t *)total,
+        hipLaunchKernelGGL(k_transform_describe, dim3(grid_for(n_poses, TR_POSES, 256 * 64)), dim3(256), transform_describe_lds_bytes(ft.n_mols, ft.n_total, n_heavy), st,
+                           frags, ft, conf_idx, rot, pos, (const int32_t *)act, n_poses, structures, (const int32_t *)d_slot, n_heavy, heavy, (const int32_t *)total,
                            nf0, nf1, basis, (const double *)(basis + size_t(KD) * (nf0 + nf1)), c->xd_D, c->xd_G, c->xd_dmax, h32);
         c->xd_valid = true, c->xd_h = n_heavy, c->xd_heavy = heavy, c->xd_h32_valid = h32 != nullptr;
         c->eb_valid = false;
     } else {
-        hipLaunchKernelGGL(k_transform, dim3(grid_for(n_poses, TR_POSES, 256 * 64)), dim3(256), transform_lds_bytes(ft.n_mols), st, frags, ft, conf_idx, rot, pos,
-                           (const int32_t *)act, int64_t(0), structures, (const int32_t *)d_slot, heavy ? n_heavy : 0, heavy, (const int32_t *)total);
+        hipLaunchKernelGGL(k_transform, dim3(grid_for(n_poses, TR_POSES, 256 * 64)), dim3(256), transform_lds_bytes(ft.n_mols, ft.n_total), st, frags, ft, conf_idx, rot, pos,
+                           (const int32_t *)act, n_poses, structures, (const int32_t *)d_slot, heavy ? n_heavy : 0, heavy, (const int32_t *)total);
     }
     TSC_HIP(hipGetLastError());
     if (n_sel_host) {
@@ -205,8 +205,8 @@
     TSC_TRY(basis_fork_launch(c, bf, s, frags, ft, conf_idx, rot, pos, d_slot, n_heavy));
     TSC_TRY(scan_mask(st, clash_mask, n_poses, bsum, nullptr, act, nullptr, total));
     TSC_TRY(read_i32_begin(c, total));
-    hipLaunchKernelGGL(k_transform, dim3(grid_for(n_poses, TR_POSES, 256 * 64)), dim3(256), transform_lds_bytes(ft.n_mols), st, frags, ft, conf_idx, rot, pos, (const int32_t *)act,
-                       int64_t(0), structures, (const int32_t *)d_slot, n_heavy, heavy, (const int32_t *)total);
+    hipLaunchKernelGGL(k_transform, dim3(grid_for(n_poses, TR_POSES, 256 * 64)), dim3(256), transform_lds_bytes(ft.n_mols, ft.n_total), st, frags, ft, conf_idx, rot, pos, (const int32_t *)act,
+                       n_poses, structures, (const int32_t *)d_slot, n_heavy, heavy, (const int32_t *)total);
     TSC_HIP(hipGetLastError());
     int32_t n_pass = 0;
     TSC_TRY(read_i32_finish(c, &n_pass));
@@ -264,14 +264,14 @@
         TSC_TRY(basis_sample_table(c, n_poses, &n_samples));
         TSC_TRY(s.get(size_t(n_samples) * n_heavy * 3, &d_sample));
         TSC_TRY(s.get(basis_doubles(n_heavy), &d_basis));
-        if (c->opt.fuse_descriptors && transform_describe_lds_bytes(ft.n_mols, n_heavy) <= 64 * 1024) {
+        if (c->opt.fuse_descriptors && transform_describe_lds_bytes(ft.n_mols, ft.n_total, n_heavy) <= 64 * 1024) {
             TSC_TRY(s.get(size_t(n_poses) * DW, &ext.D));
             TSC_TRY(s.get(size_t(n_poses), &ext.G));
             TSC_TRY(s.get(4, &ext.dmax_bits));
             if (want_heavy32(c->opt, double(n_poses) * n_heavy * 24.0))
                 TSC_TRY(s.get(size_t(n_poses) * heavy32_pitch(n_heavy), &ext.heavy32));
         }
-        fused_sample = !c->opt.deterministic_basis && sample_moments_lds_bytes(ft.n_mols, n_heavy) <= 64 * 1024;
+        fused_sample = !c->opt.deterministic_basis && sample_moments_lds_bytes(ft.n_mols, ft.n_total, n_heavy) <= 64 * 1024;
         if (fused_sample) {
             const size_t a = size_t(n_features(n_heavy, 0) + 1), b = size_t(n_features(n_heavy, 1) + 1), need = a * a + b * b;
             if (c->mom_cap < need) {
@@ -295,7 +295,7 @@
         if (fused_sample) {
             const int nf0 = n_features(n_heavy, 0), nf1 = n_features(n_heavy, 1);
             c->mom_clean = false;
-            hipLaunchKernelGGL(k_sample_moments, dim3(ceil_div(ceil_div(n_samples, TR_POSES), SM_CHUNKS), NFAM), dim3(256), sample_moments_lds_bytes(ft.n_mols, n_heavy), c->basis_stream,
+            hipLaunchKernelGGL(k_sample_moments, dim3(ceil_div(ceil_div(n_samples, TR_POSES), SM_CHUNKS), NFAM), dim3(256), sample_moments_lds_bytes(ft.n_mols, ft.n_total, n_heavy), c->basis_stream,
                                frags, ft, conf_idx, rot, pos, (const int32_t *)c->sample_dev, n_samples, (const int32_t *)d_slot, n_heavy, nf0, nf1, c->mom_acc,
                                c->mom_acc + size_t(nf0 + 1) * (nf0 + 1));
             hipLaunchKernelGGL(k_descriptor_basis, dim3(NFAM), dim3(64), 0, c->basis_stream, (const double *)c->mom_acc,
@@ -304,7 +304,7 @@
             TSC_HIP(hipGetLastError());
             c->mom_clean = true;
         } else {
-            hipLaunchKernelGGL(k_transform, dim3(grid_for(n_samples, TR_POSES, 256 * 64)), dim3(256), transform_lds_bytes(ft.n_mols), c->basis_stream, frags, ft,
+            hipLaunchKernelGGL(k_transform, dim3(grid_for(n_samples, TR_POSES, 256 * 64)), dim3(256), transform_lds_bytes(ft.n_mols, ft.n_total), c->basis_stream, frags, ft,
                                conf_idx, rot, pos, (const int32_t *)c->sample_dev, int64_t(n_samples), (double *)nullptr, (const int32_t *)d_slot, n_heavy, d_sample,
                                (const int32_t *)nullptr, d_moments, int(moment_doubles(n_heavy)));
             TSC_TRY(build_basis(c, c->basis_stream, s, d_sample, n_heavy, n_samples, 1, d_basis, ext.dmax_bits, d_moments, spread_host));
@@ -324,12 +324,12 @@
     if (ext.D) {
         const int nf0 = n_features(n_heavy, 0), nf1 = n_features(n_heavy, 1);
         TSC_HIP(hipStreamWaitEvent(st, c->ev_join, 0));
-        hipLaunchKernelGGL(k_transform_describe, dim3(grid_for(n_poses, TR_POSES, 256 * 64)), dim3(256), transform_describe_lds_bytes(ft.n_mols, n_heavy), st,
-                           frags, ft, conf_idx, rot, pos, (const int32_t *)act, structures, (const int32_t *)d_slot, n_heavy, d_heavy, (const int32_t *)total,
+        hipLaunchKernelGGL(k_transform_describe, dim3(grid_for(n_poses, TR_POSES, 256 * 64)), dim3(256), transform_describe_lds_bytes(ft.n_mols, ft.n_total, n_heavy), st,
+                           frags, ft, conf_idx, rot, pos, (const int32_t *)act, n_poses, structures, (const int32_t *)d_slot, n_heavy, d_heavy, (const int32_t *)total,
                            nf0, nf1, (const double *)d_basis, (const double *)(d_basis + size_t(KD) * (nf0 + nf1)), ext.D, ext.G, ext.dmax_bits, ext.heavy32);
     } else {
-        hipLaunchKernelGGL(k_transform, dim3(grid_for(n_poses, TR_POSES, 256 * 64)), dim3(256), transform_lds_bytes(ft.n_mols), st, frags, ft, conf_idx, rot, pos,
-                           (const int32_t *)act, int64_t(0), structures, (const int32_t *)d_slot, n_heavy, d_heavy, (const int32_t *)total);
+        hipLaunchKernelGGL(k_transform, dim3(grid_for(n_poses, TR_POSES, 256 * 64)), dim3(256), transform_lds_bytes(ft.n_mols, ft.n_total), st, frags, ft, conf_idx, rot, pos,
+                           (const int32_t *)act, n_poses, structures, (const int32_t *)d_slot, n_heavy, d_heavy, (const int32_t *)total);
     }
     TSC_HIP(hipGetLastError());
     int32_t n_pass = -1;
diff --git a/tscode_amd/csrc/sample_moments.hpp b/tscode_amd/csrc/sample_moments.hpp
--- a/tscode_amd/csrc/sample_moments.hpp
+++ b/tscode_amd/csrc/sample_moments.hpp
@@ -5,8 +5,8 @@
 namespace tsc {
 
 constexpr int SM_CHUNKS = 1;
-__host__ __device__ inline size_t sample_moments_lds_bytes(int n_mols, int h) {
-    return (transform_lds_bytes(n_mols) + 15) / 16 * 16 + size_t(TR_POSES) * (size_t(h) * 3 + size_t(h) + 1) * sizeof(double);
+__host__ __device__ inline size_t sample_moments_lds_bytes(int n_mols, int n_total, int h) {
+    return transform_lds_bytes(n_mols, n_total) + size_t(TR_POSES) * (size_t(h) * 3 + size_t(h) + 1) * sizeof(double);
 }
 inline __global__ __launch_bounds__(256) void k_sample_moments(const double *__restrict__ frags, FragTable ft, const int32_t *__restrict__ conf_idx,
                                                         const double *__restrict__ rot, const double *__restrict__ pos,
@@ -20,10 +20,14 @@
     int64_t *sP = reinterpret_cast<int64_t *>(s_tr);
     double *sR = s_tr + TR_POSES, *sT = sR + TR_POSES * nm * 9;
     int *sC = reinterpret_cast<int *>(sT + TR_POSES * nm * 3);
-    double *s_x = reinterpret_cast<double *>(s_sm_raw + (transform_lds_bytes(nm) + 15) / 16 * 16);
+    AtomEntry *tab = reinterpret_cast<AtomEntry *>(s_sm_raw + (pose_params_lds_bytes(nm) + 15) / 16 * 16);
+    double *s_x = reinterpret_cast<double *>(s_sm_raw + transform_lds_bytes(nm, n));
     double *s_n = s_x + size_t(TR_POSES) * h * 3;
     double *__restrict__ Mf = fam == 0 ? M0 : M1;
     const int n_chunks = (n_samples + TR_POSES - 1) / TR_POSES;
+    int32_t pose = sample_idx[min(int(blockIdx.x) * SM_CHUNKS * TR_POSES + tid, n_samples - 1)];
+    build_atom_table(tab, ft, heavy_slot, tid < n ? heavy_slot[tid] : -1);
+    wait_vector_loads();
     constexpr int ACC = 8;
     const bool in_regs = m * m <= 256 * ACC;
     double acc[ACC];
@@ -31,30 +35,15 @@
     for (int u = 0; u < ACC; ++u) acc[u] = 0.0;
     for (int ch = blockIdx.x * SM_CHUNKS; ch < min(n_chunks, (int(blockIdx.x) + 1) * SM_CHUNKS); ++ch) {
         const int s0 = ch * TR_POSES, ns = min(TR_POSES, n_samples - s0);
-        if (tid < ns) sP[tid] = int64_t(sample_idx[s0 + tid]);
+        if (ch > int(blockIdx.x) * SM_CHUNKS) pose = sample_idx[min(s0 + tid, n_samples - 1)];
+        if (tid < ns) sP[tid] = int64_t(pose);
         __syncthreads();
-        for (int q = tid; q < ns * nm * 9; q += 256) {
-            const int row = q / (nm * 9), w = q - row * nm * 9;
-            sR[q] = rot[sP[row] * nm * 9 + w];
-        }
-        for (int q = tid; q < ns * nm * 3; q += 256) {
-            const int row = q / (nm * 3), w = q - row * nm * 3;
-            sT[q] = pos[sP[row] * nm * 3 + w];
-        }
-        for (int q = tid; q < ns * nm; q += 256) {
-            const int row = q / nm, w = q - row * nm;
-            sC[q] = conf_idx[sP[row] * nm + w];
-        }
+        stage_pose_params(sP, sR, sT, sC, conf_idx, rot, pos, ns, nm);
         __syncthreads();
-        for (int e = tid; e < ns * n; e += 256) {
-            const int row = e / n, a = e - row * n;
-            const int hs = heavy_slot[a];
-            if (hs < 0) continue;
-            double v[3];
-            embed_atom_staged(frags, ft, sR, sT, sC, row, a, v);
+        embed_tile<4, true>(frags, tab, sR, sT, sC, ns, n, nm, [&](int row, int, int hs, const double *v) {
             double *o = s_x + (size_t(row) * h + hs) * 3;
             o[0] = v[0], o[1] = v[1], o[2] = v[2];
-        }
+        });
         __syncthreads();
         for (int e = tid; e < ns * m; e += 256) {
             const int sm = e / m, a = e - sm * m;
```

New measurement: 161.2 million (median of 6 runs). About the same (+0.9%).
